# shg8/3DGS.cpp

Measured on AMD Instinct MI355X. Metric: frames/sec at 1920×1080, 1M Gaussians, higher is better.
Workload: dtype f32

## Files before the change

3dgs.cpp_amd/binding.py:

```python
import ctypes as C
import os

import numpy as np

_HERE = os.path.dirname(os.path.abspath(__file__))
LIB_PATH = os.environ.get("GS3D_HIP_LIB", os.path.join(_HERE, "libgs3d_hip.so"))

UNIFORMS_DT = np.dtype([("camera_position", "<f4", 4), ("proj_mat", "<f4", 16), ("view_mat", "<f4", 16),
                        ("width", "<u4"), ("height", "<u4"), ("tan_fovx", "<f4"), ("tan_fovy", "<f4")])
CAMERA_DT = np.dtype([("position", "<f4", 3), ("rotation", "<f4", 4), ("fov", "<f4"),
                      ("near_plane", "<f4"), ("far_plane", "<f4")])
VERTEX_FLOATS = 60
RECORD_FLOATS = 62
BLOB_PLANES = 59


KERNEL_SOURCES = ("gs_device.h", "gs_bin.h", "gs_scene.hip", "gs_preprocess.hip", "gs_radix.hip", "gs_bin_l1.hip", "gs_bin_l2.hip",
                  "gs_blend.hip", "gs_contrib.hip", "gs_features.hip", "gs_lift.hip", "gs_kernels.h")


def library_source_hash():
    import hashlib
    import re
    h = hashlib.sha256()
    for name in KERNEL_SOURCES + ("Makefile",):
        with open(os.path.join(_HERE, "csrc", name), "r") as f:
            text = f.read()
        if name != "Makefile":
            text = re.sub(r"/\*.*?\*/", " ", text, flags=re.S)
            text = re.sub(r"//[^\n]*", " ", text)
        else:
            text = re.sub(r"#[^\n]*", " ", text)
        h.update(name.encode() + b"\0" + " ".join(text.split()).encode())
    return h.hexdigest()


STAGES = dict(tiles=(0, np.uint32), depth=(1, np.float32), radius=(2, np.float32), aabb=(3, np.uint16),
              conic_opacity=(4, np.float32), uv_rg=(5, np.float32), b=(6, np.float32),
              depth_order=(7, np.uint32), alpha_cut=(8, np.float32), sorted_tile=(11, np.uint32), sorted_gid=(12, np.uint32),
              ranges=(13, np.uint32), lists_raw=(14, np.uint32), ranges_raw=(15, np.uint32))

SYMBOLS = ["gs_last_error", "gs_device_count", "gs_read_ply", "gs_activate_records", "gs_scene_load_ply", "gs_scene_from_records",
           "gs_scene_from_vertices", "gs_scene_from_device_blob", "gs_scene_blob_floats", "gs_scene_blob",
           "gs_scene_from_device_arrays", "gs_scene_update_from_device_arrays", "gs_debug_activation_expf_scan",
           "gs_scene_transform", "gs_transform_sh_matrices", "gs_transform_camera",
           "gs_scene_num_vertices", "gs_scene_quantize_sh", "gs_scene_sh_bits", "gs_scene_download_vertex_range",
           "gs_scene_download_vertices", "gs_scene_download_cov3d",
           "gs_deactivate_vertices", "gs_write_ply", "gs_scene_to_device_arrays", "gs_scene_download_records", "gs_scene_save_ply",
           "gs_scene_destroy", "gs_renderer_create", "gs_renderer_destroy", "gs_camera_uniforms",
           "gs_render", "gs_render_host", "gs_synchronize", "gs_set_timing", "gs_set_frames_in_flight", "gs_set_sort_path", "gs_set_exp_mode", "gs_set_graph_mode", "gs_set_blend_lockstep", "gs_get_blend_lockstep", "gs_set_level1_fused", "gs_get_level1_fused", "gs_set_blend_contraction", "gs_set_antialiased", "gs_get_antialiased", "gs_get_timing_totals",
           "gs_get_frame_intervals", "gs_get_stats", "gs_poll_stats", "gs_debug_download", "gs_accumulate_contributions", "gs_blend_features", "gs_lift_pixels", "gs_debug_expf_scan", "gs_debug_alpha_cut_scan", "gs_renderer_stream",
           "gs_dist_unique_id", "gs_dist_create", "gs_dist_rank", "gs_dist_world", "gs_dist_pose_count",
           "gs_dist_broadcast_scene", "gs_dist_broadcast_scene_ex", "gs_dist_verify", "gs_dist_destroy"]


class FrameStats(C.Structure):
    _fields_ = [("num_gaussians", C.c_uint64), ("num_visible", C.c_uint64), ("num_instances", C.c_uint64),
                ("instance_capacity", C.c_uint64), ("ms_preprocess", C.c_float), ("ms_prefix_sum", C.c_float),
                ("ms_preprocess_sort", C.c_float), ("ms_sort", C.c_float), ("ms_tile_boundary", C.c_float),
                ("ms_render", C.c_float), ("ms_total", C.c_float), ("retries", C.c_uint32),
                ("num_bin_entries", C.c_uint32), ("max_bin_entries", C.c_uint32), ("sort_path", C.c_uint32),
                ("bin_tiles", C.c_uint32), ("sort_level", C.c_uint32), ("blend_redo", C.c_uint32), ("blend_resolved", C.c_uint32), ("pad_", C.c_uint32)]

    def as_dict(self):
        return {k: getattr(self, k) for k, _ in self._fields_}


def debug_alpha_cut_scan(first_bits, count, device=0):
    bad, first = C.c_uint64(0), C.c_uint32(0)
    _check(lib().gs_debug_alpha_cut_scan(C.c_int(device), C.c_uint32(first_bits), C.c_uint64(count), C.byref(bad), C.byref(first)))
    return int(bad.value), (None if bad.value == 0 else int(first.value))


def debug_expf_scan(first_bits, count, device=0):
    blocks = (count + (1 << 20) - 1) >> 20
    sums = np.zeros(blocks, np.uint64)
    guard = np.zeros(4, np.float64)
    _check(lib().gs_debug_expf_scan(C.c_int(device), C.c_uint32(first_bits), C.c_uint64(count), _p(sums), C.c_uint64(blocks), _p(guard)))
    return sums, guard


def debug_activation_expf_scan(first_bits, count, device=0):
    blocks = (count + (1 << 20) - 1) >> 20
    sums = np.zeros(blocks, np.uint64)
    _check(lib().gs_debug_activation_expf_scan(C.c_int(device), C.c_uint32(first_bits), C.c_uint64(count), _p(sums), C.c_uint64(blocks)))
    return sums


class DeviceArrays(C.Structure):
    _fields_ = [("means", C.c_void_p), ("log_scales", C.c_void_p), ("quats", C.c_void_p), ("opacity_logits", C.c_void_p),
                ("sh_dc", C.c_void_p), ("sh_rest", C.c_void_p), ("sh_rest_coeffs", C.c_uint32)]


class Transform(C.Structure):
    _fields_ = [("rotation", C.c_float * 4), ("translation", C.c_float * 3), ("scale", C.c_float)]


def _transform(rotation, translation, scale):
    t = Transform()
    t.rotation[:] = [float(v) for v in rotation]
    t.translation[:] = [float(v) for v in translation]
    t.scale = float(scale)
    return t


def _tensor_rows(name, t, trailing, device):
    if not all(hasattr(t, a) for a in ("data_ptr", "shape", "dtype", "is_contiguous", "device")):
        raise TypeError(f"{name}: a device tensor is needed (data_ptr, shape, dtype, is_contiguous, device), got {type(t).__name__}")
    if str(t.dtype).rsplit(".", 1)[-1] != "float32":
        raise TypeError(f"{name}: dtype must be float32, not {t.dtype}")
    shape = tuple(int(d) for d in t.shape)
    if len(shape) < 1:
        raise ValueError(f"{name}: shape {shape} has no row axis")
    if not t.is_contiguous():
        raise ValueError(f"{name}: the tensor must be contiguous (dense rows); call .contiguous()")
    rows, rest = shape[0], tuple(d for d in shape[1:] if d != 1) if trailing is not None else shape[1:]
    if trailing is None:
        if len(rest) != 2 or rest[1] != 3 or rest[0] not in (0, 3, 8, 15):
            raise ValueError(f"{name}: shape {shape} is not (rows, k, 3) with k in 0, 3, 8, 15")
        rows = (rows, rest[0])
    elif rest != tuple(d for d in trailing if d != 1):
        raise ValueError(f"{name}: shape {shape} is not (rows, {', '.join(map(str, trailing))})")
    dev = t.device
    kind, index = getattr(dev, "type", str(dev).split(":")[0]), getattr(dev, "index", None)
    if kind == "cpu":
        raise ValueError(f"{name}: the tensor is on the CPU; Scene.from_records takes host data")
    if (0 if index is None else int(index)) != int(device):
        raise ValueError(f"{name}: the tensor is on device {index}, the scene on device {device}")
    return rows


def _device_arrays(tensors, device, require):
    trailing = dict(means=(3,), log_scales=(3,), quats=(4,), opacity_logits=(1,), sh_dc=(3,), sh_rest=None)
# ... 417 lines not shown
        elif out is not None:
            raise ValueError("out: an output for lifted values needs values")
        l.channels = channels
        if mask is not None:
            l.mask = _tensor_exact("mask", mask, ("uint8", "bool"), (h, w), dev, owner)
        shapes = dict(out=(n, channels), weight=(n,))
        members = dict(out="out", weight="out_weight")
        result = {}
        for name, t in asked.items():
            if t is None:
                continue
            if t is True:
                import torch
                t = torch.zeros(shapes[name], dtype=torch.float64, device=f"cuda:{int(dev)}")
            setattr(l, members[name], _tensor_exact(name, t, ("float64",), shapes[name], dev, owner))
            result[name] = t
        _complete_callers_work(values, mask, *result.values())
        _check(lib().gs_lift_pixels(self._h, C.byref(l)))
        return result

    def differentiable_feature_maps(self, features):
        return _feature_maps_function().apply(self, features)

    def render_host(self, uniforms, want_rgba=True, want_bgra=False):
        h, w = int(uniforms["height"][0]), int(uniforms["width"][0])
        rgba = np.zeros((h, w, 4), np.float32) if want_rgba else None
        bgra = np.zeros((h, w, 4), np.uint8) if want_bgra else None
        _check(lib().gs_render_host(self._h, _p(uniforms), _p(rgba) if want_rgba else None,
                                    _p(bgra) if want_bgra else None))
        self._frame_hw = (h, w)
        self._frames += 1
        return rgba, bgra

    def synchronize(self):
        _check(lib().gs_synchronize(self._h))

    def set_timing(self, enabled):
        _check(lib().gs_set_timing(self._h, C.c_int(int(enabled))))

    def set_frames_in_flight(self, frames):
        _check(lib().gs_set_frames_in_flight(self._h, C.c_int(int(frames))))

    def set_exp_mode(self, mode):
        _check(lib().gs_set_exp_mode(self._h, C.c_int(int(mode))))

    def set_blend_contraction(self, enabled):
        _check(lib().gs_set_blend_contraction(self._h, C.c_int(int(bool(enabled)))))

    def set_antialiased(self, enabled):
        _check(lib().gs_set_antialiased(self._h, C.c_int(int(bool(enabled)))))

    @property
    def antialiased(self):
        rc = lib().gs_get_antialiased(self._h)
        _check(min(rc, 0))
        return bool(rc)

    def set_fast_blend(self, fast):
        self.set_exp_mode(0 if fast else 2)
        self.set_blend_contraction(bool(fast))

    def set_graph_mode(self, enabled):
        _check(lib().gs_set_graph_mode(self._h, C.c_int(int(bool(enabled)))))

    def set_blend_lockstep(self, mode):
        _check(lib().gs_set_blend_lockstep(self._h, C.c_int(int(mode))))

    def blend_lockstep(self):
        settled = C.c_int(0)
        now = lib().gs_get_blend_lockstep(self._h, C.byref(settled))
        if now < 0:
            _check(now)
        return bool(now), bool(settled.value)

    def set_level1_fused(self, mode):
        _check(lib().gs_set_level1_fused(self._h, C.c_int(int(mode))))

    def level1_fused(self):
        now = lib().gs_get_level1_fused(self._h)
        if now < 0:
            _check(now)
        return bool(now)

    def set_sort_path(self, mode):
        _check(lib().gs_set_sort_path(self._h, C.c_int(int(mode))))

    def timing_totals(self, reset=True):
        st = FrameStats()
        n = C.c_uint64()
        _check(lib().gs_get_timing_totals(self._h, C.byref(st), C.byref(n), C.c_int(int(reset))))
        return st, n.value

    def frame_intervals(self, reset=True, capacity=8192):
        out = np.zeros(capacity, np.float32)
        n = C.c_uint64()
        _check(lib().gs_get_frame_intervals(self._h, _p(out), C.c_uint64(capacity), C.byref(n), C.c_int(int(reset))))
        return out[:min(capacity, n.value)].copy()

    def stats(self):
        st = FrameStats()
        _check(lib().gs_get_stats(self._h, C.byref(st)))
        return st

    def poll_stats(self):
        st = FrameStats()
        n = C.c_uint64()
        _check(lib().gs_poll_stats(self._h, C.byref(st), C.byref(n)))
        return st, n.value

    def stage(self, name, uniforms=None):
        code, dt = STAGES[name]
        st = self.stats()
        n, v, d = st.num_gaussians, st.num_visible, min(st.num_instances, st.instance_capacity)
        count = {"tiles": n, "depth": n, "radius": n, "aabb": 4 * n, "conic_opacity": 4 * n, "uv_rg": 4 * n,
                 "b": n, "alpha_cut": n, "depth_order": v, "sorted_tile": d, "sorted_gid": d, "lists_raw": d}.get(name)
        if name in ("ranges", "ranges_raw"):
            w, h = int(uniforms["width"][0]), int(uniforms["height"][0])
            count = 2 * ((w + 15) // 16) * ((h + 15) // 16)
        out = np.zeros(max(int(count), 1), dt)
        _check(lib().gs_debug_download(self._h, C.c_int(code), _p(out), C.c_uint64(int(count) * out.itemsize)))
        return out[:int(count)]

    @property
    def stream(self):
        return lib().gs_renderer_stream(self._h)

    def close(self):
        if self._h:
            lib().gs_renderer_destroy(self._h)
            self._h = None

    def __del__(self):
        try:
            self.close()
        except Exception:
            pass


class Dist:

    ID_BYTES = 128

    @staticmethod
    def unique_id():
        buf = (C.c_uint8 * Dist.ID_BYTES)()
        _check(lib().gs_dist_unique_id(buf))
        return bytes(buf)

    def __init__(self, unique_id, rank, world, device=0):
        h = C.c_void_p()
        buf = (C.c_uint8 * Dist.ID_BYTES).from_buffer_copy(unique_id)
        _check(lib().gs_dist_create(buf, C.c_int(rank), C.c_int(world), C.c_int(device), C.byref(h)))
        self._h = h
        lib().gs_dist_pose_count.restype = C.c_uint64

    @property
    def rank(self):
        return lib().gs_dist_rank(self._h)

    @property
    def world(self):
        return lib().gs_dist_world(self._h)

    def pose_count(self, poses):
        return int(lib().gs_dist_pose_count(self._h, C.c_uint64(poses)))

    def broadcast_scene(self, scene=None, root=0, copy_on_root=False):
        out = C.c_void_p()
        _check(lib().gs_dist_broadcast_scene_ex(self._h, scene._h if scene is not None else None, C.c_int(root),
                                                C.c_uint(1 if copy_on_root else 0), C.byref(out)))
        if scene is not None and out.value == scene._h.value:
            return scene
        return Scene(out)

    def close(self):
        if self._h:
            lib().gs_dist_destroy(self._h)
            self._h = None

    def __del__(self):
        try:
            self.close()
        except Exception:
            pass
```

3dgs.cpp_amd/csrc/gs_bin.h:

```cpp
#pragma once
#include "gs_device.h"

namespace gs {


template <int R>
__device__ __forceinline__ void cover_masks(int shift, int x0, int y0, int x1, int y1, uint64_t (&m)[R]) {
    const int W = 1 << shift;
    const int rows_per_word = 64 >> shift;
    const uint64_t rowbits = x1 > x0 ? ((x1 - x0 >= 64 ? ~0ull : ((1ull << (x1 - x0)) - 1ull)) << x0) : 0ull;
#pragma unroll
    for (int r = 0; r < R; ++r) {
        uint64_t w = 0;
        for (int yy = 0; yy < rows_per_word; ++yy) {
            const int y = r * rows_per_word + yy;
            if (y >= y0 && y < y1) w |= rowbits << (yy * W);
        }
        m[r] = w;
    }
}

template <int J>
__device__ __forceinline__ uint32_t lane_xor(uint32_t x) {
    if (J == 1) return (uint32_t)__builtin_amdgcn_mov_dpp((int)x, 0xB1, 0xF, 0xF, true);
// ... 74 lines not shown
    BinGrid g;
    const uint32_t* order;
    const uint32_t* n_items;
    uint32_t n_bound;
    const uint32_t* tiles;
    const ushort4* aabb;
    const float* depth;
    const uint4* vis;
    const uint32_t* vis_count;
    uint32_t vis_region_slots;
    uint32_t* hist;
    uint32_t* bin_count;
    uint32_t* cand;
    Counters* counters;
    uint32_t capacity;
    uint32_t nblk;
    uint64_t* stamps;
};

__device__ __forceinline__ bool bin_on_screen(const BinGrid& g, uint32_t bin) {
    return (bin & ((1u << g.grid_shift) - 1u)) < g.bins_x && (bin >> g.grid_shift) < g.bins_y;
}

__device__ __forceinline__ uint32_t l1_item(const L1Args& a, uint32_t p, uint32_t n, uint32_t& box_out) {
    uint32_t gid = 0;
    box_out = 0;
    if (p < n) {
        gid = a.order ? a.order[p] : p;
        if (a.tiles[gid] != 0) {
            const ushort4 box = a.aabb[gid];
            const uint32_t x0 = box.x >> a.g.bin_shift, y0 = box.y >> a.g.bin_shift;
            const uint32_t x1 = ((box.z - 1u) >> a.g.bin_shift) + 1u, y1 = ((box.w - 1u) >> a.g.bin_shift) + 1u;
            box_out = x0 | (y0 << 8) | (x1 << 16) | (y1 << 24);
        }
    }
    return gid;
}
__device__ __forceinline__ uint32_t l1_vis_block(const L1Args& a, uint32_t blk, uint32_t& first) {
    const uint32_t per = a.vis_region_slots / kL1Items, region = blk / per, at = (blk % per) * kL1Items;
    uint32_t cnt = (uint32_t)__builtin_amdgcn_readfirstlane((int)a.vis_count[region * kVisCounterStride]);
    if (cnt > a.vis_region_slots) cnt = a.vis_region_slots;
    first = region * a.vis_region_slots + at;
    return cnt > at ? (cnt - at < (uint32_t)kL1Items ? cnt - at : (uint32_t)kL1Items) : 0u;
}
__device__ __forceinline__ uint32_t l1_bin_box(const L1Args& a, uint4 r) {
    const uint32_t x0 = (r.z & 0xFFFFu) >> a.g.bin_shift, y0 = (r.z >> 16) >> a.g.bin_shift;
    const uint32_t x1 = (((r.w & 0xFFFFu) - 1u) >> a.g.bin_shift) + 1u, y1 = (((r.w >> 16) - 1u) >> a.g.bin_shift) + 1u;
    return x0 | (y0 << 8) | (x1 << 16) | (y1 << 24);
}
template <int R>
__device__ __forceinline__ void packed_cover_masks(int shift, uint32_t box, uint64_t (&m)[R]) {
    cover_masks<R>(shift, (int)(box & 255u), (int)((box >> 8) & 255u), (int)((box >> 16) & 255u), (int)(box >> 24), m);
}

__device__ __forceinline__ uint64_t cover_word(int shift, uint32_t box, int r) {
    const int x0 = (int)(box & 255u), y0 = (int)((box >> 8) & 255u), x1 = (int)((box >> 16) & 255u), y1 = (int)(box >> 24);
    const int W = 1 << shift, rows_per_word = 64 >> shift;
    const uint64_t rowbits = x1 > x0 ? (((1ull << (x1 - x0)) - 1ull) << x0) : 0ull;
    uint64_t w = 0;
    for (int yy = 0; yy < rows_per_word; ++yy) {
        const int y = r * rows_per_word + yy;
        if (y >= y0 && y < y1) w |= rowbits << (yy * W);
    }
    return w;
}

constexpr uint32_t kL1XcdRun = 32;
__host__ __device__ constexpr uint32_t l1_grid(uint32_t nblk) {
    return (nblk + 8u * kL1XcdRun - 1u) / (8u * kL1XcdRun) * (8u * kL1XcdRun);
}
__device__ __forceinline__ uint32_t l1_block() {
    const uint32_t xcd = blockIdx.x & 7u, j = blockIdx.x >> 3;
    return ((j / kL1XcdRun) * 8u + xcd) * kL1XcdRun + j % kL1XcdRun;
}

constexpr int kCandWords = 3;
__device__ __forceinline__ uint32_t bin_local_box16(const BinGrid& g, uint32_t bin, ushort4 box) {
    const int S = 1 << g.bin_shift;
    const int ox = (int)(bin & ((1u << g.grid_shift) - 1u)) << g.bin_shift, oy = (int)(bin >> g.grid_shift) << g.bin_shift;
    const int lx0 = max((int)box.x, ox) - ox, ly0 = max((int)box.y, oy) - oy;
    const int lx1 = min((int)box.z, ox + S) - ox - 1, ly1 = min((int)box.w, oy + S) - oy - 1;
    return (uint32_t)lx0 | ((uint32_t)ly0 << 4) | ((uint32_t)lx1 << 8) | ((uint32_t)ly1 << 12);
}

}
```

3dgs.cpp_amd/csrc/gs_bin_l1.hip:

```cpp
#include "gs_bin.h"

namespace gs {

template <int R1>
__global__ __launch_bounds__(BLOCK) void k_l1_hist(L1Args a) {
    constexpr int NB = 64 * R1;
    __shared__ uint32_t s_hist[NB];
    __shared__ uint32_t s_vis;
    const int tid = threadIdx.x, lane = tid & (WAVE - 1), w = tid / WAVE;
    frame_stamp(a.stamps, ST_L1_COUNT);
    const uint32_t blk = l1_block();
    if (blk >= a.nblk) return;
    uint32_t n = a.n_items ? *a.n_items : a.n_bound;
    if (n > a.n_bound) n = a.n_bound;
    uint32_t vis_first = 0;
    const uint32_t vis_here = a.vis ? l1_vis_block(a, blk, vis_first) : 0u;
    if (a.vis && vis_here == 0) return;
    for (int b = tid; b < NB; b += BLOCK) s_hist[b] = 0;
    if (tid == 0) s_vis = 0;
    __syncthreads();
    __shared__ uint32_t s_box[kL1Chunks][WAVE];
    {
        uint32_t box[kL1PerWave];
        if (a.vis) {
// ... 183 lines not shown
            if (__builtin_amdgcn_ballot_w64(mr != 0) == 0) continue;
            walk_column(wave_transpose64(mr, lane), s_start[r * 64 + lane] + s_cnt[ch][r * 64 + lane], out, s_ids[ch]);
        }
    }
}

template <int R1>
__global__ __launch_bounds__(BLOCK) void k_l1_scatter_any_order(L1Args a) {
    constexpr int NB = 64 * R1;
    __shared__ uint32_t s_cur[NB];
    __shared__ uint32_t scratch[8];
    const int tid = threadIdx.x, lane = tid & (WAVE - 1), w = tid / WAVE;
    frame_stamp(a.stamps, ST_L1_SCATTER);
    const uint32_t blk = l1_block();
    if (blk >= a.nblk) return;
    uint32_t vis_first = 0;
    const uint32_t vis_here = a.vis ? l1_vis_block(a, blk, vis_first) : 0u;
    if (a.vis && blk != 0 && vis_here == 0) return;
    {
        uint32_t c[NB / BLOCK], sum = 0;
#pragma unroll
        for (int k = 0; k < NB / BLOCK; ++k) {
            c[k] = a.bin_count[tid * (NB / BLOCK) + k];
            sum += c[k];
        }
        uint32_t total;
        uint32_t off = block_excl_scan<BLOCK>(sum, scratch, &total);
#pragma unroll
        for (int k = 0; k < NB / BLOCK; ++k) {
            const uint32_t b = tid * (NB / BLOCK) + k;
            s_cur[b] = off + (bin_on_screen(a.g, b) ? a.hist[(size_t)b * a.nblk + blk] : 0u);
            if (blk == 0) a.bin_count[kBinOffsets + b] = off;
            off += c[k];
            if (blk == 0 && c[k]) atomicMax(&a.counters->max_bin, c[k]);
        }
        if (blk == 0 && tid == 0) {
            a.counters->bin_entries = total;
            if (total > a.capacity) atomicOr(&a.counters->overflow, 1u);
        }
    }
    uint32_t nt[kL1PerWave], key[kL1PerWave], ids[kL1PerWave];
    ushort4 tb[kL1PerWave];
    if (a.vis) {
        uint4 r[kL1PerWave];
#pragma unroll
        for (int j = 0; j < kL1PerWave; ++j) {
            const uint32_t q = (w * kL1PerWave + j) * WAVE + lane;
            r[j] = q < vis_here ? a.vis[vis_first + q] : make_uint4(0, 0, 0, 0);
        }
#pragma unroll
        for (int j = 0; j < kL1PerWave; ++j) {
            const uint32_t q = (w * kL1PerWave + j) * WAVE + lane;
            nt[j] = q < vis_here ? 1u : 0u;
            ids[j] = r[j].x;
            key[j] = r[j].y;
            tb[j] = make_ushort4((unsigned short)(r[j].z & 0xFFFFu), (unsigned short)(r[j].z >> 16), (unsigned short)(r[j].w & 0xFFFFu),
                                 (unsigned short)(r[j].w >> 16));
        }
    } else {
#pragma unroll
        for (int j = 0; j < kL1PerWave; ++j) {
            const uint32_t p = blk * kL1Items + (w * kL1PerWave + j) * WAVE + lane;
            nt[j] = p < a.n_bound ? a.tiles[p] : 0u;
            ids[j] = p;
        }
#pragma unroll
        for (int j = 0; j < kL1PerWave; ++j) {
            const uint32_t p = blk * kL1Items + (w * kL1PerWave + j) * WAVE + lane;
            tb[j] = make_ushort4(0, 0, 0, 0);
            key[j] = 0;
            if (nt[j] != 0) {
                tb[j] = a.aabb[p];
                key[j] = __float_as_uint(a.depth[p]);
            }
        }
    }
    __syncthreads();
    auto emit = [&](uint32_t bin, uint32_t k, uint32_t gid, ushort4 box) {
        const uint32_t pos = atomicAdd(&s_cur[bin], 1u);
        if (pos < a.capacity) {
            uint32_t* const rec = a.cand + (size_t)kCandWords * pos;
            rec[0] = k;
            rec[1] = gid;
            rec[2] = bin_local_box16(a.g, bin, box);
        }
    };
#pragma unroll
    for (int j = 0; j < kL1PerWave; ++j) {
        const uint32_t gid = ids[j];
        uint32_t x0 = 0, y0 = 0, x1 = 0, y1 = 0;
        if (nt[j] != 0) {
            x0 = tb[j].x >> a.g.bin_shift, y0 = tb[j].y >> a.g.bin_shift;
            x1 = ((tb[j].z - 1u) >> a.g.bin_shift) + 1u, y1 = ((tb[j].w - 1u) >> a.g.bin_shift) + 1u;
        }
        const bool big = (x1 - x0) * (y1 - y0) > kL1BigBox;
        if (!big)
            for (uint32_t y = y0; y < y1; ++y)
                for (uint32_t x = x0; x < x1; ++x) emit((y << a.g.grid_shift) | x, key[j], gid, tb[j]);
        for (uint64_t bm = __ballot(big); bm != 0; bm &= bm - 1) {
            const int src = __ffsll((unsigned long long)bm) - 1;
            const uint32_t bx0 = (uint32_t)__builtin_amdgcn_readlane((int)x0, src), by0 = (uint32_t)__builtin_amdgcn_readlane((int)y0, src);
            const uint32_t bw = (uint32_t)__builtin_amdgcn_readlane((int)x1, src) - bx0;
            const uint32_t cells = bw * ((uint32_t)__builtin_amdgcn_readlane((int)y1, src) - by0);
            const uint32_t bkey = (uint32_t)__builtin_amdgcn_readlane((int)key[j], src);
            const uint32_t bgid = (uint32_t)__builtin_amdgcn_readlane((int)gid, src);
            const uint32_t blo = (uint32_t)__builtin_amdgcn_readlane((int)((uint32_t)tb[j].x | ((uint32_t)tb[j].y << 16)), src);
            const uint32_t bhi = (uint32_t)__builtin_amdgcn_readlane((int)((uint32_t)tb[j].z | ((uint32_t)tb[j].w << 16)), src);
            const ushort4 bbox = make_ushort4((unsigned short)(blo & 0xFFFFu), (unsigned short)(blo >> 16), (unsigned short)(bhi & 0xFFFFu),
                                              (unsigned short)(bhi >> 16));
            for (uint32_t c = lane; c < cells; c += WAVE) emit(((by0 + c / bw) << a.g.grid_shift) | (bx0 + c % bw), bkey, bgid, bbox);
        }
    }
}

__global__ __launch_bounds__(BLOCK) void k_vis_to_planes(const uint4* __restrict__ vis, const uint32_t* __restrict__ vis_count,
                                                         uint32_t region_slots, uint32_t* __restrict__ tiles, float* __restrict__ depth,
                                                         ushort4* __restrict__ aabb) {
    const uint32_t region = blockIdx.y, slot = blockIdx.x * BLOCK + threadIdx.x;
    const uint32_t count = min(vis_count[region * kVisCounterStride + 1], region_slots);
    if (slot >= count) return;
    const uint4 e = vis[(size_t)region * region_slots + slot];
    const uint32_t x0 = e.z & 0xFFFFu, y0 = e.z >> 16, x1 = e.w & 0xFFFFu, y1 = e.w >> 16;
    tiles[e.x] = (x1 - x0) * (y1 - y0);
    depth[e.x] = __uint_as_float(e.y);
    aabb[e.x] = make_ushort4((unsigned short)x0, (unsigned short)y0, (unsigned short)x1, (unsigned short)y1);
}
void launch_vis_to_planes(const AttrView& av, uint32_t n, hipStream_t s) {
    if (!av.vis || n == 0) return;
    (void)hipMemsetAsync(av.tiles, 0, (size_t)n * sizeof(uint32_t), s);
    hipLaunchKernelGGL(k_vis_to_planes, dim3((av.vis_region_slots + BLOCK - 1) / BLOCK, kVisRegions), dim3(BLOCK), 0, s, av.vis, av.vis_count,
                       av.vis_region_slots, av.tiles, av.depth, av.aabb);
}

static L1Args l1_args(const BinLaunch& b) {
    L1Args a;
    a.g = BinGrid{b.tiles_x, b.tiles_y, b.bins_x, b.bins_y, b.bin_shift, b.grid_shift};
    a.order = b.order;
    a.n_items = b.n_items;
    a.n_bound = b.n_bound;
    a.tiles = b.tiles;
    a.aabb = b.aabb;
    a.depth = b.depth;
    a.vis = b.vis;
    a.vis_count = b.vis_count;
    a.vis_region_slots = b.vis_region_slots;
    a.hist = b.hist;
    a.bin_count = b.bin_count;
    a.cand = b.cand;
    a.counters = b.counters;
    a.capacity = b.cand_capacity;
    a.nblk = b.vis ? kVisRegions * (b.vis_region_slots / kL1Items) : bin_level1_blocks(b.n_bound);
    a.stamps = b.stamps;
    return a;
}

uint32_t bin_level1_blocks(uint32_t n_items) { return (n_items + kL1Items - 1) / kL1Items; }
uint32_t vis_region_slots(uint32_t n) {
    const uint32_t groups = (n + BLOCK - 1) / BLOCK, per_region = (groups + kVisRegions - 1) / kVisRegions;
    const uint32_t slots = per_region * BLOCK;
    return slots == 0 ? kL1Items : (slots + kL1Items - 1) / kL1Items * kL1Items;
}
uint32_t bin_level1_columns(uint32_t n_items) {
    const uint32_t dense = kVisRegions * (vis_region_slots(n_items) / kL1Items), planes = bin_level1_blocks(n_items);
    return dense > planes ? dense : planes;
}
static_assert(BLOCK >= (int)kVisRegions, "k_blend's first workgroup zeroes the list counters, k_l1_scan's sums them: a thread each");

// ... 22 lines not shown
```

3dgs.cpp_amd/csrc/gs_bin_l2.hip:

```cpp
#include "gs_bin.h"

namespace gs {

struct SlabDesc {
    uint32_t off, c_total;
    uint32_t kmin;
    int32_t sh;
    uint32_t b_lo, b_hi;
    uint32_t ready;
    uint32_t pad;
    uint32_t cur[64];
};
static_assert(sizeof(SlabDesc) == 288, "descriptor layout");

struct BuildArgs {
    BinGrid g;
    uint32_t* cand;
    const uint32_t* bin_count;
    const float* depth;
    const ushort4* aabb;
    uint32_t* ranges;
    uint32_t* sorted_gid;
    Counters* counters;
    uint32_t capacity;
    uint32_t cand_capacity;
    SlabDesc* slabs;
    uint32_t slab_capacity;
    uint32_t epoch;
    uint64_t* stamps;
    const uint32_t* l1_words;
    uint32_t l1_cap;
};

__device__ __forceinline__ uint32_t bin_candidates(const BuildArgs& a, uint32_t bin) {
    return a.l1_words ? a.l1_words[(size_t)(kL1FusedCursor0 + bin) * kL1FusedStride] : a.bin_count[bin];
}
__device__ __forceinline__ uint32_t bin_offset(const BuildArgs& a, uint32_t bin) {
    return a.l1_words ? ((bin >> a.g.grid_shift) * a.g.bins_x + (bin & ((1u << a.g.grid_shift) - 1u))) * a.l1_cap : a.bin_count[kBinOffsets + bin];
}
__device__ __forceinline__ void bin_close_one_pass(const BuildArgs& a, uint32_t& c, int tid) {
    if (!a.l1_words) return;
    if (tid == 0 && c != 0) {
        atomicAdd(&a.counters->bin_entries, c);
        atomicMax(&a.counters->max_bin, c);
    }
    if (c > a.l1_cap) {
        if (tid == 0) atomicOr(&a.counters->overflow, 1u);
        c = 0;
    }
}
__device__ __forceinline__ void one_pass_visible(const BuildArgs& a) {
    if (!a.l1_words || blockIdx.x != 0 || threadIdx.x >= kVisRegions) return;
    uint32_t v = a.l1_words[(size_t)threadIdx.x * kL1FusedStride];
    for (int o = WAVE / 2; o != 0; o >>= 1) v += (uint32_t)__shfl_xor((int)v, o);
    if ((threadIdx.x & (WAVE - 1)) == 0 && v != 0) atomicAdd(&a.counters->visible, v);
}

__device__ __forceinline__ uint32_t bin_local_box(const BinGrid& g, uint32_t bin, ushort4 box) {
    const int S = 1 << g.bin_shift;
    const int ox = (int)(bin & ((1u << g.grid_shift) - 1u)) << g.bin_shift, oy = (int)(bin >> g.grid_shift) << g.bin_shift;
    const int lx0 = max((int)box.x, ox) - ox, ly0 = max((int)box.y, oy) - oy;
    const int lx1 = min((int)box.z, ox + S) - ox, ly1 = min((int)box.w, oy + S) - oy;
    return (uint32_t)lx0 | ((uint32_t)ly0 << 8) | ((uint32_t)lx1 << 16) | ((uint32_t)ly1 << 24);
}

constexpr int kBuildSlots = 16;

#ifdef GS_BUILD_TIMING
__device__ unsigned long long g_build_t[1024][10];
#define BUILD_ROW(v) uint32_t build_row = (v)
#define BUILD_ROW_SET(v) build_row = (v)
#define BUILD_T(i) do { if (threadIdx.x == 0) g_build_t[build_row][i] = wall_clock64(); } while (0)
#else
#define BUILD_ROW(v) do { } while (0)
#define BUILD_ROW_SET(v) do { } while (0)
#define BUILD_T(i) do { } while (0)
#endif

template <int R2, int THREADS, bool SORT>
struct BuildLayout {
    static constexpr int NW = THREADS / WAVE;
    static constexpr int MAXC = SORT ? THREADS * 16 : 0;
    static constexpr int SS = 64 * R2;
    static constexpr bool CACHE_BOX = SORT && R2 <= 4;
    static constexpr int TABLES = 3 * SS + kBuildSlots * SS / 2 + (SORT ? 0 : kBuildSlots * WAVE);
    static constexpr int WCNT = SORT ? NW * 256 : 0;
    static constexpr int T_OFF = (SORT && (CACHE_BOX || TABLES > MAXC)) ? 2 * MAXC : 0;
    static constexpr int WORDS = (T_OFF + TABLES > 2 * MAXC + WCNT) ? T_OFF + TABLES : 2 * MAXC + WCNT;
};

template <int R2, int THREADS, bool SORT>
__global__ __launch_bounds__(THREADS) void k_bin_build(BuildArgs a) {
    frame_stamp(a.stamps, ST_L2);
    one_pass_visible(a);
    BUILD_ROW(blockIdx.x);
    using L = BuildLayout<R2, THREADS, SORT>;
    constexpr int NW = L::NW, MAXC = L::MAXC, SS = L::SS, PER = kBuildSlots / NW;
    extern __shared__ uint32_t smem[];
    uint32_t* const s_key = smem;
    uint32_t* const s_id = smem + MAXC;
    uint32_t (*const s_wcnt)[256] = reinterpret_cast<uint32_t(*)[256]>(smem + 2 * MAXC);
    uint32_t* const t_cnt = smem + L::T_OFF;
    uint32_t* const t_cur = t_cnt + SS;
    uint16_t (*const r_cnt)[SS] = reinterpret_cast<uint16_t(*)[SS]>(t_cnt + 3 * SS);
    uint32_t* const w_ids = t_cnt + 3 * SS + kBuildSlots * SS / 2;
    __shared__ uint32_t scratch[NW];
    __shared__ uint32_t s_seg;

    const int tid = threadIdx.x, lane = tid & (WAVE - 1), w = tid / WAVE;
    const uint32_t bin = ((blockIdx.x / a.g.bins_x) << a.g.grid_shift) | (blockIdx.x % a.g.bins_x);
    BUILD_T(0);
    uint32_t c, off;
    c = bin_candidates(a, bin);
    off = bin_offset(a, bin);
// ... 198 lines not shown
    for (uint32_t rb = 0; rb < nch; rb += kBuildSlots, par ^= 1) {
        uint64_t col[PER][R2];
#pragma unroll
        for (int j = 0; j < PER; ++j) {
            const int slot = w * PER + j;
            uint32_t gid;
            chunk_columns(rb + slot, col[j], gid);
#pragma unroll
            for (int r = 0; r < R2; ++r) r_cnt[slot][r * 64 + lane] = (uint16_t)__popcll(col[j][r]);
            if (!SORT) w_ids[slot * WAVE + lane] = gid;
        }
        __syncthreads();
        for (int t = tid; t < SS; t += THREADS) {
            uint32_t run = 0;
#pragma unroll
            for (int k = 0; k < kBuildSlots; ++k) {
                const uint32_t v = r_cnt[k][t];
                r_cnt[k][t] = (uint16_t)run;
                run += v;
            }
            t_cur[(par ^ 1) * SS + t] = t_cur[par * SS + t] + run;
        }
        __syncthreads();
#pragma unroll
        for (int j = 0; j < PER; ++j) {
            const int slot = w * PER + j;
            const uint32_t ch = rb + slot;
            const uint32_t* ids = SORT ? s_id + (ch < nch ? ch : 0u) * WAVE : w_ids + slot * WAVE;
#pragma unroll
            for (int r = 0; r < R2; ++r) {
                if (__builtin_amdgcn_ballot_w64(col[j][r] != 0) == 0) continue;
                walk_column(col[j][r], t_cur[par * SS + r * 64 + lane] + r_cnt[slot][r * 64 + lane], out, ids);
            }
        }
    }
    BUILD_T(7);
}

#ifdef GS_BUILD_TIMING
extern "C" int gs_debug_build_timing(unsigned long long* out ) {
    return hipMemcpyFromSymbol(out, HIP_SYMBOL(g_build_t), sizeof(unsigned long long) * 1024 * 10) == hipSuccess ? 0 : -1;
}
#endif

__device__ __forceinline__ __amdgpu_buffer_rsrc_t uniform_rsrc(const void* p, uint32_t bytes) {
    const uint64_t addr = reinterpret_cast<uint64_t>(p);
    const uint32_t lo = (uint32_t)__builtin_amdgcn_readfirstlane((int)(uint32_t)addr);
    const uint32_t hi = (uint32_t)__builtin_amdgcn_readfirstlane((int)(uint32_t)(addr >> 32));
    return __builtin_amdgcn_make_buffer_rsrc(reinterpret_cast<void*>(((uint64_t)hi << 32) | lo), 0,
                                             __builtin_amdgcn_readfirstlane((int)bytes), 0x27000);
}

__device__ __forceinline__ uint32_t cover16(uint32_t pb) {
    const uint32_t lx0 = pb & 15u, ly0 = (pb >> 4) & 15u, lx1 = (pb >> 8) & 15u, ly1 = (pb >> 12) & 15u;
    const uint32_t xm = ((2u << lx1) - (1u << lx0)) & 15u;
    const uint32_t rows = (16u << (4u * ly1)) - (1u << (4u * ly0));
    return (xm * 0x1111u) & rows;
}

template <int ROUNDS>
struct FastLayout {
    static constexpr int THREADS = 1024, NW = THREADS / WAVE, MAXC = THREADS * ROUNDS;
    static constexpr int WCNT_WORDS = NW * 512 / 2;
    static constexpr int MISC_WORDS = 64 + 64 + NW * 64;
    static constexpr int TAIL = WCNT_WORDS > MISC_WORDS ? WCNT_WORDS : MISC_WORDS;
    static constexpr int WORDS = 2 * MAXC + TAIL;
};

template <int ROUNDS, int MODE = 0>
__device__ __forceinline__ void bin_fast_body(const BuildArgs& a) {
    constexpr bool SLABS = MODE != 0;
    using L = FastLayout<ROUNDS>;
    constexpr int THREADS = L::THREADS, NW = L::NW, MAXC = L::MAXC;
    extern __shared__ uint32_t smem[];
    uint32_t* const s_pay = smem;
    uint32_t* const s_key = smem + MAXC;
    uint16_t (*const s_wcnt)[512] = reinterpret_cast<uint16_t(*)[512]>(smem + 2 * MAXC);
    uint32_t* const s_id = smem + MAXC;
    uint16_t* const s_box = reinterpret_cast<uint16_t*>(smem);
    uint16_t (*const s_tbl)[64] = reinterpret_cast<uint16_t(*)[64]>(smem + MAXC / 2);
    uint32_t* const t_cnt = smem + 2 * MAXC;
    uint32_t* const t_cur = t_cnt + 64;
    uint32_t (*const s_seg)[64] = reinterpret_cast<uint32_t(*)[64]>(t_cnt + 128);
    __shared__ uint32_t scratch[NW], scratch_hi[NW];
    __shared__ uint32_t s_seg0, s_flag;
    constexpr int kSlotBits = SLABS ? 16 : 14;
    constexpr uint32_t kSlotMask = (1u << kSlotBits) - 1u;
    constexpr uint32_t kMaxInBin = SLABS ? 65535u : (uint32_t)MAXC;
    constexpr int kMaxSlabs = 16;
    __shared__ uint32_t g_cur[SLABS ? 64 : 1], t_tot[SLABS ? 64 : 1];
    __shared__ uint32_t slab_first[SLABS ? kMaxSlabs + 1 : 1];
    __shared__ uint32_t cnt2[(MODE == 1 || MODE == 3) ? kMaxSlabs : 1][64];
    __shared__ uint32_t s_fill;
    __shared__ uint16_t q_order[MODE == 3 ? 1024 : 1];
    __shared__ uint32_t q_item, q_planned;

    BUILD_ROW(MODE == 2 ? 1023u : blockIdx.x);
    if constexpr (MODE != 2) frame_stamp(a.stamps, ST_L2);
    if constexpr (MODE != 2) one_pass_visible(a);
    int tid = threadIdx.x, lane = tid & (WAVE - 1), w = tid / WAVE;
    auto screen_bin = [&](uint32_t i) { return ((i / a.g.bins_x) << a.g.grid_shift) | (i % a.g.bins_x); };
    uint32_t bin = screen_bin(MODE == 3 ? 0u : blockIdx.x);
    bool slab_item = MODE == 2;
    BUILD_T(0);
    uint32_t c_total = 0, off = 0;
    auto bin_extent = [&]() {
        c_total = (uint32_t)__builtin_amdgcn_readfirstlane((int)bin_candidates(a, bin));
        off = (uint32_t)__builtin_amdgcn_readfirstlane((int)bin_offset(a, bin));
        bin_close_one_pass(a, c_total, tid);
        if ((uint64_t)off + c_total > a.cand_capacity) c_total = 0;
        if (c_total > kMaxInBin) {
            if (tid == 0) atomicOr(&a.counters->overflow, 2u);
            c_total = 0;
        }
    };
    if constexpr (MODE == 0 || MODE == 1) bin_extent();
    if (tid == 0) s_flag = 0;
    BUILD_T(1);
#define multi (MODE == 2 ? true : (MODE == 1 ? c_total > (uint32_t)MAXC : (MODE == 3 ? (slab_item || c_total > (uint32_t)MAXC) : false)))
    uint32_t c = multi ? 0u : c_total;
    int rounds = (int)((c + THREADS - 1) / THREADS);
    typedef uint32_t u32x3 __attribute__((ext_vector_type(3)));
#define recs uniform_rsrc(a.cand + (size_t)kCandWords * off, c_total * 12u)
    uint64_t lt_mask = (1ull << lane) - 1ull;
    uint32_t wbase = (uint32_t)w * (uint32_t)rounds * WAVE;
    auto refresh = [&]() {
        int t = threadIdx.x;
        asm volatile("" : "+v"(t));
        tid = t;
        lane = t & (WAVE - 1);
        w = t / WAVE;
        lt_mask = (1ull << lane) - 1ull;
        wbase = (uint32_t)w * (uint32_t)rounds * WAVE;
    };
    auto radix_pass = [&](int shift, int db, uint32_t sub) {
        const uint32_t dmask = (1u << db) - 1u;
        for (int k = tid; k < NW * 512 / 2; k += THREADS) reinterpret_cast<uint32_t*>(&s_wcnt[0][0])[k] = 0;
        __syncthreads();
        uint32_t key[ROUNDS], pay[ROUNDS], rank[ROUNDS];
#pragma unroll
        for (int r = 0; r < ROUNDS; ++r) {
            key[r] = 0;
            pay[r] = 0;
            rank[r] = 0;
            if (r < rounds) {
                const uint32_t e = wbase + r * WAVE + lane;
                const bool ok = e < c;
                if (ok) {
                    key[r] = s_key[e] - sub;
                    pay[r] = s_pay[e];
                }
                const uint32_t d = (key[r] >> shift) & dmask;
                const uint64_t okm = __ballot(ok);
                uint32_t mlo = (uint32_t)okm, mhi = (uint32_t)(okm >> 32);
#pragma unroll
                for (int bit = 0; bit < 9; ++bit) {
                    if (bit < db) {
                        const uint32_t mine = (d >> bit) & 1u;
                        const uint64_t b = __builtin_amdgcn_ballot_w64(mine != 0);
                        const uint32_t splat = 0u - mine;
                        mlo &= ~((uint32_t)b ^ splat);
                        mhi &= ~((uint32_t)(b >> 32) ^ splat);
                    }
                }
                const uint64_t m = ((uint64_t)mhi << 32) | mlo;
                uint32_t old = 0;
                const int leader = m ? (__ffsll((unsigned long long)m) - 1) : 0;
                if (ok && lane == leader) {
                    old = s_wcnt[w][d];
                    s_wcnt[w][d] = (uint16_t)(old + (uint32_t)__popcll(m));
                }
                old = __shfl(old, leader, WAVE);
                rank[r] = old + (uint32_t)__popcll(m & lt_mask);
            }
        }
        __syncthreads();
        {
            uint32_t cw[NW], cnt = 0;
            if (tid < 512) {
#pragma unroll
                for (int k = 0; k < NW; ++k) {
                    cw[k] = s_wcnt[k][tid];
                    cnt += cw[k];
                }
            }
            uint32_t all;
            uint32_t excl = block_excl_scan<THREADS>(cnt, scratch, &all);
            if (tid < 512) {
#pragma unroll
                for (int k = 0; k < NW; ++k) {
                    s_wcnt[k][tid] = (uint16_t)excl;
                    excl += cw[k];
                }
            }
        }
        __syncthreads();
#pragma unroll
        for (int r = 0; r < ROUNDS; ++r) {
            if (r < rounds) {
                const uint32_t e = wbase + r * WAVE + lane;
                if (e < c) {
                    const uint32_t d = (key[r] >> shift) & dmask;
                    const uint32_t pos = (uint32_t)s_wcnt[w][d] + rank[r];
                    s_key[pos] = key[r];
                    s_pay[pos] = pay[r];
                }
            }
        }
        __syncthreads();
    };
    auto block_minmax = [&](uint32_t lo, uint32_t hi, uint32_t& kmin, uint32_t& span) {
#pragma unroll
        for (int d = 1; d < WAVE; d <<= 1) {
            lo = min(lo, (uint32_t)__shfl_xor((int)lo, d, WAVE));
            hi = max(hi, (uint32_t)__shfl_xor((int)hi, d, WAVE));
        }
        __syncthreads();
        if (lane == 0) {
            scratch[w] = lo;
            scratch_hi[w] = hi;
        }
        __syncthreads();
#pragma unroll
        for (int k = 0; k < NW; ++k) {
            lo = min(lo, scratch[k]);
            hi = max(hi, scratch_hi[k]);
        }
        kmin = (uint32_t)__builtin_amdgcn_readfirstlane((int)lo);
        span = (uint32_t)__builtin_amdgcn_readfirstlane((int)hi) - kmin;
    };
    auto key_range = [&](uint32_t& kmin, uint32_t& span) {
        uint32_t lo = 0xFFFFFFFFu, hi = 0u;
#pragma unroll
        for (int r = 0; r < ROUNDS; ++r) {
            const uint32_t e = r * THREADS + tid;
            if (r < rounds && e < c) {
                const uint32_t k = s_key[e];
                lo = min(lo, k);
                hi = max(hi, k);
            }
        }
        block_minmax(lo, hi, kmin, span);
    };
    auto sort_by_key_lsd = [&](uint32_t kmin, uint32_t span) {
        const int bits = span ? 32 - __builtin_clz(span) : 0;
        const int npass = (bits + 8) / 9;
        const int db = npass ? (bits + npass - 1) / npass : 0;
#pragma unroll 1
        for (int pass = 0; pass < npass; ++pass) radix_pass(pass * db, db, pass == 0 ? kmin : 0u);
        return npass ? kmin : 0u;
    };
    constexpr uint32_t kMsdBuckets = 4096, kMsdBucketMax = 64;
    uint32_t* const m_cnt = smem + 2 * MAXC;
    uint16_t* const m_start = reinterpret_cast<uint16_t*>(smem + 2 * MAXC + kMsdBuckets / 2);
    static_assert(kMsdBuckets * 4 <= L::TAIL * 4, "the bucket tables live in the counters' area");
    auto sort_by_key_msd = [&](uint32_t kmin, uint32_t span) -> bool {
        const int bits = 32 - __builtin_clz(span);
        const int sh = bits > 12 ? bits - 12 : 0;
        for (uint32_t k = tid; k < kMsdBuckets / 2; k += THREADS) m_cnt[k] = 0;
        __syncthreads();
        uint32_t key[ROUNDS], pay[ROUNDS];
#pragma unroll
        for (int r = 0; r < ROUNDS; ++r) {
            const uint32_t e = r * THREADS + tid;
            key[r] = 0;
            pay[r] = 0;
            if (r < rounds && e < c) {
                key[r] = s_key[e];
                pay[r] = s_pay[e];
                const uint32_t b = (key[r] - kmin) >> sh;
                atomicAdd(&m_cnt[b >> 1], 1u << (16u * (b & 1u)));
            }
        }
        __syncthreads();
        {
            const uint2 w2 = reinterpret_cast<const uint2*>(m_cnt)[tid];
            const uint32_t v0 = w2.x & 0xFFFFu, v1 = w2.x >> 16, v2 = w2.y & 0xFFFFu, v3 = w2.y >> 16;
            uint32_t all;
            uint32_t excl = block_excl_scan<THREADS>(v0 + v1 + v2 + v3, scratch, &all);
            if (max(max(v0, v1), max(v2, v3)) > kMsdBucketMax) s_flag = 2;
            reinterpret_cast<uint2*>(m_cnt)[tid] = make_uint2(0u, 0u);
            ushort4 st;
            st.x = (unsigned short)excl;
            st.y = (unsigned short)(excl + v0);
            st.z = (unsigned short)(excl + v0 + v1);
            st.w = (unsigned short)(excl + v0 + v1 + v2);
            reinterpret_cast<ushort4*>(m_start)[tid] = st;
        }
        __syncthreads();
        if (__builtin_amdgcn_readfirstlane((int)s_flag) == 2) {
            __syncthreads();
            if (tid == 0) s_flag = 0;
            return false;
        }
#pragma unroll
        for (int r = 0; r < ROUNDS; ++r) {
            const uint32_t e = r * THREADS + tid;
            if (r < rounds && e < c) {
                const uint32_t b = (key[r] - kmin) >> sh;
                const uint32_t old = atomicAdd(&m_cnt[b >> 1], 1u << (16u * (b & 1u)));
                const uint32_t pos = (uint32_t)m_start[b] + ((old >> (16u * (b & 1u))) & 0xFFFFu);
                s_key[pos] = key[r];
                s_pay[pos] = pay[r];
            }
        }
        __syncthreads();
        uint32_t dst[ROUNDS];
#pragma unroll
        for (int r = 0; r < ROUNDS; ++r) {
            const uint32_t e = r * THREADS + tid;
            dst[r] = 0xFFFFFFFFu;
            if (r < rounds && e < c) {
                const uint32_t k = s_key[e];
                pay[r] = s_pay[e];
                key[r] = k;
                const uint32_t b = (k - kmin) >> sh;
                const uint32_t j0 = m_start[b], j1 = b + 1 < kMsdBuckets ? (uint32_t)m_start[b + 1] : c;
                uint32_t before = 0;
                for (uint32_t j = j0; j < j1; ++j) {
                    const uint32_t kj = s_key[j];
                    before += (kj < k || (kj == k && j < e)) ? 1u : 0u;
                }
                dst[r] = j0 + before;
            }
        }
        __syncthreads();
#pragma unroll
        for (int r = 0; r < ROUNDS; ++r)
            if (dst[r] != 0xFFFFFFFFu) {
                s_key[dst[r]] = key[r];
                s_pay[dst[r]] = pay[r];
            }
        __syncthreads();
        return true;
    };
    auto sort_by_key = [&](bool try_msd) -> uint32_t {
        uint32_t kmin, span;
        key_range(kmin, span);
        if (span == 0) return 0u;
        if constexpr (ROUNDS <= 12) {
            if (try_msd && sort_by_key_msd(kmin, span)) return 0u;
        }
        return sort_by_key_lsd(kmin, span);
    };
    const int S = 1 << a.g.bin_shift;
    auto place_lists = [&](uint32_t v, uint32_t* cursors) {
        uint32_t d_bin;
        const uint32_t excl = block_excl_scan<THREADS>(v, scratch, &d_bin);
        if (tid == 0) {
            const uint32_t seg = d_bin ? atomicAdd(&a.counters->instances, d_bin) : 0u;
            s_seg0 = seg;
            if ((uint64_t)seg + d_bin > a.capacity) atomicOr(&a.counters->overflow, 1u);
        }
        __syncthreads();
        if (tid < 64) {
            const uint32_t ox = (bin & ((1u << a.g.grid_shift) - 1u)) << a.g.bin_shift, oy = (bin >> a.g.grid_shift) << a.g.bin_shift;
            const uint32_t lx = (uint32_t)tid & (uint32_t)(S - 1), ly = (uint32_t)tid >> a.g.bin_shift;
            const uint32_t x = ox + lx, y = oy + ly;
            const uint64_t start64 = (uint64_t)s_seg0 + excl;
            const uint32_t start = start64 > a.capacity ? a.capacity : (uint32_t)start64;
            const uint32_t end = start64 + v > a.capacity ? a.capacity : (uint32_t)(start64 + v);
            if (ly < (uint32_t)S && x < a.g.tiles_x && y < a.g.tiles_y) {
                a.ranges[2 * (y * a.g.tiles_x + x)] = v ? start : 0u;
                a.ranges[2 * (y * a.g.tiles_x + x) + 1] = v ? end : 0u;
            }
            cursors[tid] = start;
        }
    };
    uint32_t n_slabs = 1, g_kmin = 0;
    int g_sh = 0;
    auto plan_bin = [&]() {
    if constexpr (MODE == 1 || MODE == 3) if (!slab_item && multi) {
        uint32_t lo = 0xFFFFFFFFu, hi = 0u;
        for (uint32_t base = 0; base < c_total; base += 8 * THREADS) {
            uint32_t k[8];
#pragma unroll
            for (int r = 0; r < 8; ++r) k[r] = __builtin_amdgcn_raw_buffer_load_b32(recs, (base + r * THREADS + tid) * 12u, 0, 0);
#pragma unroll
            for (int r = 0; r < 8; ++r)
                if (base + r * THREADS + tid < c_total) {
                    lo = min(lo, k[r]);
                    hi = max(hi, k[r]);
                }
        }
        uint32_t span;
        block_minmax(lo, hi, g_kmin, span);
        const int bits = span ? 32 - __builtin_clz(span) : 0;
        g_sh = bits > 12 ? bits - 12 : 0;
        for (uint32_t k = tid; k < kMsdBuckets / 2; k += THREADS) m_cnt[k] = 0;
        for (uint32_t k = tid; k < (uint32_t)kMaxSlabs * 64u; k += THREADS) cnt2[k >> 6][k & 63u] = 0;
        __syncthreads();
        for (uint32_t base = 0; base < c_total; base += 8 * THREADS) {
            uint32_t k[8];
#pragma unroll
            for (int r = 0; r < 8; ++r) k[r] = __builtin_amdgcn_raw_buffer_load_b32(recs, (base + r * THREADS + tid) * 12u, 0, 0);
#pragma unroll
            for (int r = 0; r < 8; ++r)
                if (base + r * THREADS + tid < c_total) {
                    const uint32_t bk = (k[r] - g_kmin) >> g_sh;
                    atomicAdd(&m_cnt[bk >> 1], 1u << (16u * (bk & 1u)));
                }
        }
        __syncthreads();
        {
            const uint2 w2 = reinterpret_cast<const uint2*>(m_cnt)[tid];
            const uint32_t v0 = w2.x & 0xFFFFu, v1 = w2.x >> 16, v2 = w2.y & 0xFFFFu, v3 = w2.y >> 16;
            uint32_t all;
            const uint32_t excl = block_excl_scan<THREADS>(v0 + v1 + v2 + v3, scratch, &all);
            if (max(max(v0, v1), max(v2, v3)) > (uint32_t)MAXC) s_flag = 3;
            ushort4 st;
            st.x = (unsigned short)excl;
            st.y = (unsigned short)(excl + v0);
            st.z = (unsigned short)(excl + v0 + v1);
            st.w = (unsigned short)(excl + v0 + v1 + v2);
            reinterpret_cast<ushort4*>(m_start)[tid] = st;
            if (tid == 0) {
                slab_first[0] = 0;
                s_fill = 1;
            }
        }
        __syncthreads();
        for (int k = 0; k < kMaxSlabs; ++k) {
            const uint32_t base = m_start[slab_first[k]];
            if (c_total - base <= (uint32_t)MAXC) break;
#pragma unroll
            for (int j = 0; j < 4; ++j) {
                const uint32_t bk = 4u * tid + j;
                const uint32_t p0 = m_start[bk], p1 = bk + 1 < kMsdBuckets ? (uint32_t)m_start[bk + 1] : c_total;
                if (p0 - base <= (uint32_t)MAXC && p1 - base > (uint32_t)MAXC && bk > slab_first[k]) {
                    slab_first[k + 1] = bk;
                    s_fill = k + 2;
                }
            }
            __syncthreads();
            if (s_fill != (uint32_t)k + 2) {
// ... 59 lines not shown
        }
        __syncthreads();
        place_lists(tid < 64 ? t_tot[tid] : 0u, g_cur);
        __syncthreads();
        if (tid == 0) {
            const uint32_t base = n_slabs ? atomicAdd(&a.counters->slabs, n_slabs) : 0u;
            s_seg0 = base;
            if (base + n_slabs > a.slab_capacity) atomicOr(&a.counters->overflow, 2u);
        }
        __syncthreads();
        const uint32_t dbase = (uint32_t)__builtin_amdgcn_readfirstlane((int)s_seg0);
        if (dbase + n_slabs <= a.slab_capacity) {
            auto put = [&](uint32_t* p, uint32_t v) {
                if constexpr (MODE == 3) __hip_atomic_store(p, v, __ATOMIC_RELAXED, __HIP_MEMORY_SCOPE_AGENT);
                else *p = v;
            };
            for (uint32_t k = 0; k < n_slabs; ++k) {
                SlabDesc* d = a.slabs + dbase + k;
                if (tid < 64) put(&d->cur[tid], g_cur[tid] + cnt2[k][tid]);
                if (tid == 64) {
                    put(&d->off, off);
                    put(&d->c_total, c_total);
                    put(&d->kmin, g_kmin);
                    put(reinterpret_cast<uint32_t*>(&d->sh), (uint32_t)g_sh);
                    put(&d->b_lo, slab_first[k]);
                    put(&d->b_hi, slab_first[k + 1]);
                }
            }
            if constexpr (MODE == 3) {
                asm volatile("s_waitcnt vmcnt(0)" ::: "memory");
                __syncthreads();
                if (tid == 0) {
                    for (uint32_t k = 0; k < n_slabs; ++k)
                        __hip_atomic_store(&a.slabs[dbase + k].ready, a.epoch, __ATOMIC_RELAXED, __HIP_MEMORY_SCOPE_AGENT);
                    asm volatile("s_waitcnt vmcnt(0)" ::: "memory");
                }
            }
        }
        n_slabs = 0;
    }
    };
    if constexpr (MODE == 1) plan_bin();
    auto slab_body = [&](const uint32_t slab) {
    if constexpr (SLABS) if (multi) {
        const uint32_t b_lo = slab_first[slab], b_hi = slab_first[slab + 1];
        __syncthreads();
        if (tid == 0) s_fill = 0;
        __syncthreads();
        for (uint32_t base = 0; base < c_total; base += 8 * THREADS) {
            uint32_t k[8], bx[8];
#pragma unroll
            for (int r = 0; r < 8; ++r) {
                const u32x3 rec = __builtin_amdgcn_raw_buffer_load_b96(recs, (base + r * THREADS + tid) * 12u, 0, 0);
                k[r] = rec.x;
                bx[r] = rec.z;
            }
#pragma unroll
            for (int r = 0; r < 8; ++r) {
                const uint32_t e = base + r * THREADS + tid;
                const uint32_t bk = (k[r] - g_kmin) >> g_sh;
                const bool mine = e < c_total && bk >= b_lo && bk < b_hi;
                const uint64_t mm = __builtin_amdgcn_ballot_w64(mine);
                if (mm != 0) {
                    uint32_t at = 0;
                    if (lane == __ffsll((unsigned long long)mm) - 1) at = atomicAdd(&s_fill, (uint32_t)__popcll(mm));
                    at = (uint32_t)__builtin_amdgcn_readlane((int)at, __ffsll((unsigned long long)mm) - 1) + (uint32_t)__popcll(mm & lt_mask);
                    if (mine && at < (uint32_t)MAXC) {
                        s_key[at] = k[r];
                        s_pay[at] = e | (bx[r] << kSlotBits);
                    }
                }
            }
        }
        __syncthreads();
        c = min((uint32_t)__builtin_amdgcn_readfirstlane((int)s_fill), (uint32_t)MAXC);
        rounds = (int)((c + THREADS - 1) / THREADS);
        wbase = (uint32_t)w * (uint32_t)rounds * WAVE;
    }
    for (int attempt = 0; c != 0 && attempt < 2; ++attempt) {
        uint32_t tid12 = (uint32_t)tid * 12u;
        asm volatile("" : "+v"(tid12));
        constexpr int HR = ROUNDS <= 8 ? ROUNDS : ROUNDS / 2;
        const int h_end = multi ? 0 : ROUNDS;
#pragma unroll
        for (int h = 0; h < h_end; h += HR) {
            uint32_t k[HR], b[HR];
#pragma unroll
            for (int r = 0; r < HR; ++r) {
                k[r] = 0;
                b[r] = 0;
                if (h + r < rounds) {
                    const u32x3 rec = __builtin_amdgcn_raw_buffer_load_b96(recs, tid12 + (uint32_t)(h + r) * (THREADS * 12u), 0, 0);
                    k[r] = rec.x;
                    b[r] = rec.z;
                }
            }
#pragma unroll
            for (int r = 0; r < HR; ++r) {
                const uint32_t e = (h + r) * THREADS + tid;
                if (h + r < rounds && e < c) {
                    s_key[e] = k[r];
                    s_pay[e] = e | (b[r] << kSlotBits);
                }
            }
        }
        if (attempt == 0) BUILD_T(2);
        sort_by_key(attempt == 0);
        if (attempt == 0) BUILD_T(8);
        refresh();
        uint32_t my_id[ROUNDS], run_len[(ROUNDS + 3) / 4];
        bool too_long = false;
#pragma unroll
        for (int q = 0; q < (ROUNDS + 3) / 4; ++q) run_len[q] = 0;
#pragma unroll
        for (int r = 0; r < ROUNDS; ++r) {
            const uint32_t e = r * THREADS + tid;
            my_id[r] = 0;
            if (r < rounds && e < c) {
                my_id[r] = __builtin_amdgcn_raw_buffer_load_b32(recs, (s_pay[e] & kSlotMask) * 12u + 4u, 0, 0);
                const uint32_t k = s_key[e];
                if (attempt == 0 && (e == 0 || s_key[e - 1] != k) && e + 1 < c && s_key[e + 1] == k) {
                    uint32_t more = 1;
                    while (e + more + 1 < c && more < 64 && s_key[e + more + 1] == k) ++more;
                    if (e + more + 1 < c && s_key[e + more + 1] == k) too_long = true;
                    run_len[r / 4] |= more << (8 * (r % 4));
                }
            }
        }
        if (too_long) s_flag = 1;
        __syncthreads();
        const bool redo = __builtin_amdgcn_readfirstlane((int)s_flag) != 0;
#pragma unroll
        for (int r = 0; r < ROUNDS; ++r) {
            const uint32_t e = r * THREADS + tid;
            if (r < rounds && e < c) s_id[e] = my_id[r];
        }
        __syncthreads();
        if (attempt == 0) BUILD_T(9);
        if (multi && redo) {
            if (tid == 0) atomicOr(&a.counters->overflow, 2u);
            __syncthreads();
            if (tid == 0) s_flag = 0;
            break;
        }
        if (!redo) {
#pragma unroll
            for (int r = 0; r < ROUNDS; ++r) {
                const uint32_t more = (run_len[r / 4] >> (8 * (r % 4))) & 255u;
                if (more != 0) {
                    const uint32_t e = r * THREADS + tid;
                    for (uint32_t i = e + 1; i <= e + more; ++i) {
                        const uint32_t vi = s_id[i], vp = s_pay[i];
                        uint32_t j = i;
                        while (j > e && s_id[j - 1] > vi) {
                            s_id[j] = s_id[j - 1];
                            s_pay[j] = s_pay[j - 1];
                            --j;
                        }
                        s_id[j] = vi;
                        s_pay[j] = vp;
                    }
                }
            }
            __syncthreads();
            break;
        }
        const uint32_t id_base = sort_by_key(false);
        uint32_t nk[ROUNDS], ni[ROUNDS], nb[ROUNDS];
#pragma unroll
        for (int r = 0; r < ROUNDS; ++r) {
            const uint32_t e = r * THREADS + tid;
            nk[r] = ni[r] = nb[r] = 0;
            if (r < rounds && e < c) {
                const uint32_t pw = s_pay[e];
                nk[r] = __builtin_amdgcn_raw_buffer_load_b32(recs, (pw & kSlotMask) * 12u, 0, 0);
                ni[r] = s_id[e] + id_base;
                nb[r] = pw >> kSlotBits;
            }
        }
        __syncthreads();
#pragma unroll
        for (int r = 0; r < ROUNDS; ++r) {
            const uint32_t e = r * THREADS + tid;
            if (r < rounds && e < c) {
                u32x3 rec = {nk[r], ni[r], nb[r]};
                __builtin_amdgcn_raw_buffer_store_b96(rec, recs, e * 12u, 0, 0);
            }
        }
        __threadfence_block();
        if (tid == 0) s_flag = 0;
        __syncthreads();
    }
#undef recs
    BUILD_T(3);
    refresh();
    const uint32_t nch = (c + WAVE - 1) / WAVE;
    {
        uint32_t pb16[ROUNDS];
#pragma unroll
        for (int r = 0; r < ROUNDS; ++r) {
            const uint32_t e = r * THREADS + tid;
            pb16[r] = e < c ? s_pay[e] >> kSlotBits : 0u;
        }
        __syncthreads();
        for (uint32_t k = tid; k < (uint32_t)MAXC / 2; k += THREADS) smem[MAXC / 2 + k] = 0;
        if (tid < 64) t_cnt[tid] = 0;
        __syncthreads();
#pragma unroll
        for (int r = 0; r < ROUNDS; ++r) {
            const uint32_t e = r * THREADS + tid;
            const uint32_t pb = pb16[r];
            if (e < c) s_box[e] = (uint16_t)pb;
            if (S == 4) {
                const uint32_t ch = (uint32_t)r * NW + (uint32_t)__builtin_amdgcn_readfirstlane(w);
                if (ch < nch) {
                    const uint32_t cm = e < c ? cover16(pb) : 0u;
                    uint32_t mine = 0;
#pragma unroll
                    for (int t = 0; t < 16; ++t) {
                        const uint64_t bal = __builtin_amdgcn_ballot_w64(((cm >> t) & 1u) != 0);
                        mine = lane == t ? (uint32_t)__popcll(bal) : mine;
                    }
                    s_tbl[ch][lane] = (uint16_t)mine;
                }
            }
        }
        if (S != 4) {
            __syncthreads();
            for (uint32_t ch = w; ch < nch; ch += NW) {
                const uint32_t e = ch * WAVE + lane;
                const uint32_t pb = e < c ? (uint32_t)s_box[e] : 0xFFFFu;
                uint64_t m[1];
                cover_masks<1>(3, (int)(pb & 15u), (int)((pb >> 4) & 15u), (int)((pb >> 8) & 15u) + 1, (int)(pb >> 12) + 1, m);
                if (e >= c) m[0] = 0;
                s_tbl[ch][lane] = (uint16_t)__popcll(wave_transpose64(m[0], lane));
            }
        }
    }
    __syncthreads();
    BUILD_T(4);
    {
        const int t = tid & 63, g = tid >> 6;
        const uint32_t per = (nch + NW - 1) / NW;
        const uint32_t q0 = min(nch, (uint32_t)g * per), q1 = min(nch, q0 + per);
        uint32_t sum = 0;
        for (uint32_t q = q0; q < q1; ++q) sum += s_tbl[q][t];
        s_seg[g][t] = sum;
        __syncthreads();
        if (tid < 64) {
            uint32_t run = 0;
#pragma unroll
            for (int k = 0; k < NW; ++k) {
                const uint32_t v = s_seg[k][tid];
                s_seg[k][tid] = run;
                run += v;
            }
            t_cnt[tid] = run;
        }
        __syncthreads();
        uint32_t run = s_seg[g][t];
// ... 163 lines not shown
    BUILD_T(7);
}
#undef multi
template <int ROUNDS> __global__ void k_bin_fast(BuildArgs a);
template <> __global__ __launch_bounds__(1024, 4) void k_bin_fast<4>(BuildArgs a) { bin_fast_body<4>(a); }
template <> __global__ __launch_bounds__(1024, 4) void k_bin_fast<8>(BuildArgs a) { bin_fast_body<8>(a); }
template <> __global__ __launch_bounds__(1024, 4) void k_bin_fast<12>(BuildArgs a) { bin_fast_body<12>(a); }
template <> __global__ __launch_bounds__(1024, 4) void k_bin_fast<16>(BuildArgs a) { bin_fast_body<16>(a); }
constexpr int kSlabRounds = 12;
__global__ __launch_bounds__(1024, 4) void k_bin_slabs(BuildArgs a) { bin_fast_body<kSlabRounds, 1>(a); }
__global__ __launch_bounds__(1024, 4) void k_slab_work(BuildArgs a) { bin_fast_body<kSlabRounds, 2>(a); }
__global__ __launch_bounds__(1024, 4) void k_bin_queue(BuildArgs a) { bin_fast_body<kSlabRounds, 3>(a); }

template <int R2, int THREADS, bool SORT>
static hipError_t build_prepare() {
    return hipFuncSetAttribute(reinterpret_cast<const void*>(&k_bin_build<R2, THREADS, SORT>),
                               hipFuncAttributeMaxDynamicSharedMemorySize,
                               (int)(BuildLayout<R2, THREADS, SORT>::WORDS * sizeof(uint32_t)));
}
template <int ROUNDS>
static hipError_t fast_prepare() {
    return hipFuncSetAttribute(reinterpret_cast<const void*>(&k_bin_fast<ROUNDS>), hipFuncAttributeMaxDynamicSharedMemorySize,
                               (int)(FastLayout<ROUNDS>::WORDS * sizeof(uint32_t)));
}
void bin_debug_occupancy() {
    int n4 = -1, n8 = -1, n16 = -1;
    (void)hipOccupancyMaxActiveBlocksPerMultiprocessor(&n4, reinterpret_cast<const void*>(&k_bin_fast<4>), 1024,
                                                       FastLayout<4>::WORDS * sizeof(uint32_t));
    (void)hipOccupancyMaxActiveBlocksPerMultiprocessor(&n8, reinterpret_cast<const void*>(&k_bin_fast<8>), 1024,
                                                       FastLayout<8>::WORDS * sizeof(uint32_t));
    (void)hipOccupancyMaxActiveBlocksPerMultiprocessor(&n16, reinterpret_cast<const void*>(&k_bin_fast<16>), 1024,
                                                       FastLayout<16>::WORDS * sizeof(uint32_t));
    hipFuncAttributes a4{}, a8{};
    (void)hipFuncGetAttributes(&a4, reinterpret_cast<const void*>(&k_bin_fast<4>));
    (void)hipFuncGetAttributes(&a8, reinterpret_cast<const void*>(&k_bin_fast<8>));
    std::fprintf(stderr, "[occupancy] k_bin_fast<4>: %d blocks/CU (regs %d, static lds %zu, dyn %zu); <8>: %d (regs %d); <16>: %d\n", n4,
                 a4.numRegs, a4.sharedSizeBytes, FastLayout<4>::WORDS * sizeof(uint32_t), n8, a8.numRegs, n16);
}

hipError_t bin_prepare_device() {
    hipError_t e = build_prepare<4, 1024, true>();
    if (e == hipSuccess) e = build_prepare<16, 1024, true>();
    if (e == hipSuccess) e = fast_prepare<8>();
    if (e == hipSuccess) e = fast_prepare<12>();
    if (e == hipSuccess) e = fast_prepare<16>();
    if (e == hipSuccess)
        e = hipFuncSetAttribute(reinterpret_cast<const void*>(&k_bin_slabs), hipFuncAttributeMaxDynamicSharedMemorySize,
                                (int)(FastLayout<kSlabRounds>::WORDS * sizeof(uint32_t)));
    if (e == hipSuccess)
        e = hipFuncSetAttribute(reinterpret_cast<const void*>(&k_slab_work), hipFuncAttributeMaxDynamicSharedMemorySize,
                                (int)(FastLayout<kSlabRounds>::WORDS * sizeof(uint32_t)));
    if (e == hipSuccess)
        e = hipFuncSetAttribute(reinterpret_cast<const void*>(&k_bin_queue), hipFuncAttributeMaxDynamicSharedMemorySize,
                                (int)(FastLayout<kSlabRounds>::WORDS * sizeof(uint32_t)));
    return e;
}

template <int R2>
static void launch_build(const BuildArgs& a, bool sort, uint32_t bins, hipStream_t s) {
    constexpr size_t lds1 = BuildLayout<R2, 1024, true>::WORDS * sizeof(uint32_t);
    constexpr size_t lds2 = BuildLayout<R2, 1024, false>::WORDS * sizeof(uint32_t);
    if (sort) hipLaunchKernelGGL((k_bin_build<R2, 1024, true>), dim3(bins), dim3(1024), lds1, s, a);
    else hipLaunchKernelGGL((k_bin_build<R2, 1024, false>), dim3(bins), dim3(1024), lds2, s, a);
}

void launch_bin_level2(const BinLaunch& b, int level, hipStream_t s) {
    BuildArgs a;
    a.g = BinGrid{b.tiles_x, b.tiles_y, b.bins_x, b.bins_y, b.bin_shift, b.grid_shift};
    a.cand = b.cand;
    a.bin_count = b.bin_count;
    a.depth = b.depth;
    a.aabb = b.aabb;
    a.ranges = b.ranges;
    a.sorted_gid = b.sorted_gid;
    a.counters = b.counters;
    a.capacity = b.capacity;
    a.cand_capacity = b.cand_capacity;
    a.slabs = reinterpret_cast<SlabDesc*>(b.slabs);
    a.slab_capacity = b.slab_capacity;
    a.epoch = b.slab_epoch;
    a.stamps = b.stamps;
    a.l1_words = b.l1_fused_words;
    a.l1_cap = b.l1_fused_cap;
    const uint32_t bins = b.bins_x * b.bins_y;
    const bool sort = level < kBinSortLevels;
    if (sort && b.bin_shift <= 3) {
        if (level == 0) hipLaunchKernelGGL(k_bin_fast<4>, dim3(bins), dim3(1024), FastLayout<4>::WORDS * sizeof(uint32_t), s, a);
        else if (level == 1) hipLaunchKernelGGL(k_bin_fast<8>, dim3(bins), dim3(1024), FastLayout<8>::WORDS * sizeof(uint32_t), s, a);
        else if (level == 2) hipLaunchKernelGGL(k_bin_fast<12>, dim3(bins), dim3(1024), FastLayout<12>::WORDS * sizeof(uint32_t), s, a);
        else if (level == 3) hipLaunchKernelGGL(k_bin_fast<16>, dim3(bins), dim3(1024), FastLayout<16>::WORDS * sizeof(uint32_t), s, a);
        else if (b.slab_epoch != 0) {
            hipLaunchKernelGGL(k_bin_queue, dim3(bins < kQueueWorkGroups ? bins : kQueueWorkGroups), dim3(1024), FastLayout<kSlabRounds>::WORDS * sizeof(uint32_t), s, a);
        } else {
            hipLaunchKernelGGL(k_bin_slabs, dim3(bins), dim3(1024), FastLayout<kSlabRounds>::WORDS * sizeof(uint32_t), s, a);
            hipLaunchKernelGGL(k_slab_work, dim3(kSlabWorkGroups), dim3(1024), FastLayout<kSlabRounds>::WORDS * sizeof(uint32_t), s, a);
        }
    } else if (b.bin_shift <= 3) {
        launch_build<1>(a, sort, bins, s);
    } else if (b.bin_shift == 4) {
        launch_build<4>(a, sort, bins, s);
    } else {
        launch_build<16>(a, sort, bins, s);
    }
}
}
```

3dgs.cpp_amd/csrc/gs_kernels.h:

```cpp
#pragma once
#include <hip/hip_runtime.h>
#include <stdint.h>

#include "../../include/gs3d_hip.h"
#include "gs_levels.h"

namespace gs {

constexpr int kSortTileKeys = 2048;
constexpr int kSortMaxBlocks = 1024;

enum ScenePlane { P_POS = 0, P_SCALE = 3, P_ROT = 6, P_OPACITY = 10, P_SH = 11, P_COUNT = 59 };
constexpr uint64_t blob_stride(uint64_t n) { return (n + 15) & ~uint64_t(15); }
constexpr uint64_t blob_floats(uint64_t n) { return P_SH * blob_stride(n) + 48 * n; }

struct SceneView {
    const float* blob;
    const float* cov3d;
    uint32_t n;
    uint32_t stride;
    const uint16_t* sh16;
    const float* acut;
    const uint32_t* perm;
};

struct AttrRecord {
    float4 conic_op;
    float4 uv_rg;
    float4 b_cut_r;
    float4 depth_radius;
};
static_assert(sizeof(AttrRecord) == 64, "one line per Gaussian");

struct AttrView {
    uint32_t* tiles;
    float* depth;
    ushort4* aabb;
    AttrRecord* rec;
    uint4* vis;
    uint32_t* vis_count;
    uint32_t vis_region_slots;
};
constexpr uint32_t kVisRegions = 256, kVisCounterStride = 32;
uint32_t vis_region_slots(uint32_t n);

constexpr uint32_t kL1FusedStride = 32, kL1FusedCursor0 = kVisRegions, kL1FusedWords = (kVisRegions + 1024) * kL1FusedStride;
struct L1Fused {
    uint32_t* words;
    uint32_t* cand;
    uint32_t cap;
    uint64_t* vis_mask;
    uint32_t tiles_x, tiles_y, bins_x, bins_y;
    int bin_shift, grid_shift;
};

struct Counters {
    uint32_t visible;
    uint32_t instances;
    uint32_t overflow;
    uint32_t bin_entries;
    uint32_t max_bin;
    uint32_t slabs;
    uint32_t blend_resolved;
    uint32_t blend_redo;
    uint32_t q_head, q_bins_done;
};
enum FrameStamp { ST_PREPROCESS = 0, ST_ORDER = 1, ST_L1_COUNT = 2, ST_L1_SCATTER = 3, ST_L2 = 4, ST_BLEND = 5, ST_END = 6, ST_COUNT = 8 };

struct FrameParams {
    gs_uniforms u;
    float* rgba;
    uint8_t* bgra;
    Counters* host_counters;
    uint64_t* host_stamps;
};

constexpr int kBinSortMax = 16384;
constexpr uint32_t kSlabDescBytes = 288, kSlabCapacity = 8192, kSlabWorkGroups = 512, kQueueWorkGroups = 256;

void launch_cov3d(const float* blob, float* cov3d, uint32_t n, uint32_t stride, uint32_t first, uint32_t count, hipStream_t s);
void launch_alpha_cut(const float* blob, float* cut, uint32_t n, uint32_t stride, uint32_t* beyond_unit, hipStream_t s);
void launch_permute_blob(const float* src, const uint32_t* perm, float* dst, uint32_t n, uint32_t stride, hipStream_t s);
void launch_blob_checksum(const float* blob, uint64_t floats, uint64_t* out, hipStream_t s);
void launch_sh_to_half(const float* blob, uint16_t* sh16, uint32_t stride, uint32_t first, uint32_t count, hipStream_t s);
void launch_ingest_arrays(const gs_device_arrays& a, float* blob, uint32_t stride, uint32_t first, uint32_t count, bool replace_rest,
                          hipStream_t s);
struct SceneTransform {
    float R[9];
    float t[3];
    float s;
    float q[4];
    float M[9 + 25 + 49];
};
void launch_scene_transform(const SceneTransform& x, float* blob, uint32_t stride, uint32_t first, uint32_t count, hipStream_t s);
void launch_scene_export(const gs_device_arrays_out& a, const float* blob, uint32_t stride, uint32_t first, uint32_t count, hipStream_t s);
void launch_scene_export_records(float* records, const float* blob, uint32_t stride, uint32_t first, uint32_t count, hipStream_t s);
void launch_preprocess(const SceneView& sv, const gs_uniforms& u, const AttrView& av, Counters* counters,
                       const FrameParams* fp, uint64_t* stamps, bool antialiased, const L1Fused& lf, hipStream_t s);
void launch_frame_end(uint64_t* stamps, uint64_t* host_stamps, const FrameParams* fp, uint32_t* l1_words, uint32_t l1_counters, hipStream_t s);

struct RadixPass {
    const uint32_t* keys_in;
    const uint32_t* vals_in;
    uint32_t* keys_out;
    uint32_t* vals_out;
    const uint32_t* n_in;
    uint32_t n_static;
    const uint32_t* tiles;
    uint32_t* n_out;
    uint32_t* block_hist;
    uint32_t* digit_total;
    int shift;
    int bits;
    int blocks;
    int first;
    uint64_t* stamps;
};
void launch_radix_pass(const RadixPass& p, hipStream_t s);

struct BinLaunch {
    const uint32_t* order;
    const uint32_t* n_items;
    uint32_t n_bound;
    const uint32_t* tiles;
    const ushort4* aabb;
    const float* depth;
    const uint4* vis;
    uint32_t* vis_count;
    uint32_t vis_region_slots;
    uint32_t* hist;
    uint32_t* bin_count;
    uint32_t* cand;
    uint32_t* ranges;
    uint32_t* sorted_gid;
    Counters* counters;
    uint32_t capacity;
    uint32_t cand_capacity;
    const uint32_t* l1_fused_words;
    uint32_t l1_fused_cap;
    void* slabs;
    uint32_t slab_capacity;
    uint32_t slab_epoch;
    uint32_t tiles_x, tiles_y, bins_x, bins_y;
    int bin_shift;
    int grid_shift;
    uint64_t* stamps;
};
void launch_vis_to_planes(const AttrView& av, uint32_t n, hipStream_t s);
void launch_records_to_planes(const uint64_t* vis_mask, const uint32_t* perm, const AttrView& av, uint32_t n, uint32_t width, uint32_t height,
                              hipStream_t s);
uint32_t bin_level1_blocks(uint32_t n_items);
uint32_t bin_level1_columns(uint32_t n_items);
void bin_debug_occupancy();
hipError_t bin_prepare_device();
void launch_bin_level1_count(const BinLaunch& b, hipStream_t s);
void launch_bin_level1_scatter(const BinLaunch& b, bool any_order, hipStream_t s);
void launch_bin_level2(const BinLaunch& b, int level, hipStream_t s);

void launch_blend(const uint32_t* ranges, const uint32_t* sorted_gid, const uint32_t* tile_order, const AttrView& av,
                  uint32_t width,
                  uint32_t height, float* rgba, uint8_t* bgra, Counters* counters,
                  Counters* host_counters ,
                  int exp_mode ,
                  bool contract ,
                  const FrameParams* fp,
                  bool lockstep ,
                  uint64_t* stamps ,
                  hipStream_t s);

void launch_contributions(const uint32_t* ranges, const uint32_t* sorted_gid, const uint32_t* tile_order, const AttrRecord* rec,
                          uint32_t width, uint32_t height, const uint8_t* mask, uint64_t* weight, uint32_t* pixels, uint32_t* top_id,
                          hipStream_t s);

constexpr int kFeatureGroup = 16;
void launch_features(const uint32_t* ranges, const uint32_t* sorted_gid, const uint32_t* tile_order, const AttrRecord* rec,
                     uint32_t width, uint32_t height, const float* features, uint32_t channels, float* out_features, float* out_alpha,
                     float* out_depth, float* out_median, hipStream_t s);

constexpr int kLiftGroup = 16, kLiftGroupSmall = 4;
void launch_lift(const uint32_t* ranges, const uint32_t* sorted_gid, const uint32_t* tile_order, const AttrRecord* rec, uint32_t width,
                 uint32_t height, const uint8_t* mask, const float* values, uint32_t channels, double* out, double* out_weight,
                 hipStream_t s);

}
```

3dgs.cpp_amd/csrc/gs_preprocess.hip:

```cpp
#include "gs_bin.h"

namespace gs {

constexpr float SH_C0 = 0.28209479177387814f;
constexpr float SH_C1 = 0.4886025119029199f;

__device__ __forceinline__ float ndc2pix(float v, int S) { return ((v + 1.0f) * (float)S - 1.0f) * 0.5f; }

struct PreUniforms {
    gs_uniforms u;
    Counters* counters;
    const FrameParams* fp;
    uint64_t* stamps;
};

template <int R1>
struct PreBins {
    uint32_t tbl[R1 ? 64 * R1 : 1];
    uint32_t vis;
};

constexpr int kPrePlane = 68, kPreStage = 4 * kPrePlane + 16;
constexpr int kPreShHalf = 32;
constexpr int kPreWaveLds = kPreShHalf * 12 + 4;
static_assert(kPreWaveLds >= kPreStage, "the record stage must fit the wave's LDS slab");

template <class SH>
__device__ __forceinline__ void sh_to_rgb(const SH& S, float x, float y, float z, float (&rgb)[3]) {
    const float C2_0 = 1.0925484305920792f, C2_1 = -1.0925484305920792f, C2_2 = 0.31539156525252005f,
                C2_3 = -1.0925484305920792f, C2_4 = 0.5462742152960396f;
    const float C3_0 = -0.5900435899266435f, C3_1 = 2.890611442640554f, C3_2 = -0.4570457994644658f,
                C3_3 = 0.3731763325901154f, C3_4 = -0.4570457994644658f, C3_5 = 1.445305721320277f,
                C3_6 = -0.5900435899266435f;
    float c[3];
#define GS_SH_FENCE() asm volatile("" : "+v"(c[0]), "+v"(c[1]), "+v"(c[2]) :: "memory")
#pragma unroll
    for (int k = 0; k < 3; ++k) c[k] = SH_C0 * S(0, k);
#pragma unroll
    for (int k = 0; k < 3; ++k) c[k] -= SH_C1 * S(1, k) * y;
#pragma unroll
    for (int k = 0; k < 3; ++k) c[k] += SH_C1 * S(2, k) * z;
#pragma unroll
    for (int k = 0; k < 3; ++k) c[k] -= SH_C1 * S(3, k) * x;
    GS_SH_FENCE();
#pragma unroll
    for (int k = 0; k < 3; ++k) c[k] += C2_0 * S(4, k) * x * y;
#pragma unroll
    for (int k = 0; k < 3; ++k) c[k] += C2_1 * S(5, k) * y * z;
#pragma unroll
    for (int k = 0; k < 3; ++k) c[k] += C2_2 * S(6, k) * (2.0f * z * z - x * x - y * y);
#pragma unroll
    for (int k = 0; k < 3; ++k) c[k] += C2_3 * S(7, k) * z * x;
    GS_SH_FENCE();
#pragma unroll
    for (int k = 0; k < 3; ++k) c[k] += C2_4 * S(8, k) * (x * x - y * y);
#pragma unroll
    for (int k = 0; k < 3; ++k) c[k] += C3_0 * S(9, k) * (3.0f * x * x - y * y) * y;
#pragma unroll
    for (int k = 0; k < 3; ++k) c[k] += C3_1 * S(10, k) * x * y * z;
#pragma unroll
    for (int k = 0; k < 3; ++k) c[k] += C3_2 * S(11, k) * (4.0f * z * z - x * x - y * y) * y;
    GS_SH_FENCE();
#pragma unroll
    for (int k = 0; k < 3; ++k) c[k] += C3_3 * S(12, k) * z * (2.0f * z * z - 3.0f * x * x - 3.0f * y * y);
#pragma unroll
    for (int k = 0; k < 3; ++k) c[k] += C3_4 * S(13, k) * x * (4.0f * z * z - x * x - y * y);
#pragma unroll
    for (int k = 0; k < 3; ++k) c[k] += C3_5 * S(14, k) * (x * x - y * y) * z;
#pragma unroll
    for (int k = 0; k < 3; ++k) c[k] += C3_6 * S(15, k) * x * (x * x - 3.0f * y * y);
#pragma unroll
    for (int k = 0; k < 3; ++k) rgb[k] = c[k] + 0.5f;
#undef GS_SH_FENCE
    if (rgb[0] < 0.0f) rgb[0] = 0.0f;
}
struct ShFromLds {
    const float* p;
    __device__ __forceinline__ float operator()(int j, int k) const { return p[j * 3 + k]; }
};
struct ShFromLds16 {
    const uint16_t* p;
    __device__ __forceinline__ float operator()(int j, int k) const { return __half2float(__ushort_as_half(p[j * 3 + k])); }
};
// ... 140 lines not shown
        {
            const uint32_t x0 = bb & 255u, y0 = (bb >> 8) & 255u, x1 = (bb >> 16) & 255u, y1 = bb >> 24;
            const bool big = (x1 - x0) * (y1 - y0) > kL1BigBox;
            if (!big)
                for (uint32_t y = y0; y < y1; ++y)
                    for (uint32_t x = x0; x < x1; ++x) atomicAdd(&bins.tbl[(y << lf.grid_shift) | x], 1u);
            for (uint64_t bm = __ballot(big); bm != 0; bm &= bm - 1) {
                const uint32_t b1 = (uint32_t)__builtin_amdgcn_readlane((int)bb, __ffsll((unsigned long long)bm) - 1);
                const uint32_t gx0 = b1 & 255u, gy0 = (b1 >> 8) & 255u, bw = ((b1 >> 16) & 255u) - gx0, cells = bw * ((b1 >> 24) - gy0);
                for (uint32_t c = lane; c < cells; c += WAVE) atomicAdd(&bins.tbl[((gy0 + c / bw) << lf.grid_shift) | (gx0 + c % bw)], 1u);
            }
            const uint32_t nv = (uint32_t)__popcll(__ballot(vis));
            if (lane == 0 && nv) atomicAdd(&bins.vis, nv);
        }
        __syncthreads();
#pragma unroll
        for (int k = 0; k < NB / BLOCK; ++k) {
            const uint32_t b = (uint32_t)(k * BLOCK + tid), cnt = bins.tbl[b];
            fbase[k] = cnt ? atomicAdd(lf.words + (size_t)(kL1FusedCursor0 + b) * kL1FusedStride, cnt) : 0u;
        }
        if (tid == 0 && bins.vis)
            __hip_atomic_fetch_add(lf.words + (size_t)((i / BLOCK) % kVisRegions) * kL1FusedStride, bins.vis, __ATOMIC_RELAXED, __HIP_MEMORY_SCOPE_AGENT);
    }

    float rgb[3] = {0.0f, 0.0f, 0.0f};
    const uint64_t vm_sh = __ballot(vis);
    const uint32_t n_vis = (uint32_t)__popcll(vm_sh);
    const uint32_t my_rank = (uint32_t)__popcll(vm_sh & ((1ull << lane) - 1ull));
    uint8_t* const s_src = reinterpret_cast<uint8_t*>(stage + kPreShHalf * 12);
    if (vis) s_src[my_rank] = (uint8_t)lane;
    __builtin_amdgcn_wave_barrier();
    const int chunks = sv.sh16 ? 6 : 12;
    const uint32_t per_inst = sv.sh16 ? 10u : 5u;
    const uint32_t slot = sv.sh16 ? lane / 6u : lane / 12u, q = sv.sh16 ? lane % 6u : lane % 12u;
    const char* const sh_bytes = sv.sh16 ? reinterpret_cast<const char*>(sv.sh16) : reinterpret_cast<const char*>(blob + (size_t)P_SH * N);
    const size_t sh_stride = sv.sh16 ? 96 : 192;
    const uint32_t lds_base = (uint32_t)__builtin_amdgcn_readfirstlane((int)(uint32_t)(uintptr_t)stage);
    for (uint32_t half = 0; half * kPreShHalf < n_vis; ++half) {
        const uint32_t first = half * kPreShHalf, last = min(n_vis, first + (uint32_t)kPreShHalf);
        uint32_t dst = lds_base;
        for (uint32_t g0 = first; g0 < last; g0 += per_inst, dst += per_inst * (uint32_t)sh_stride) {
            const uint32_t g = g0 + slot;
            if (lane < 60u && g < last) {
                const uint32_t src_lane = s_src[g];
                const char* gsrc = sh_bytes + (size_t)(i - lane + src_lane) * sh_stride + q * 16u;
                unsigned keep;
                asm volatile("s_mov_b32 %0, m0\n\ts_mov_b32 m0, %2\n\ts_nop 0\n\tglobal_load_lds_dwordx4 %1, off\n\ts_mov_b32 m0, %0"
                             : "=&s"(keep) : "v"(gsrc), "s"(dst) : "memory");
            }
        }
        asm volatile("s_waitcnt vmcnt(0)" ::: "memory");
        __builtin_amdgcn_wave_barrier();
        if (vis && my_rank >= first && my_rank < last) {
            float dx = px - u.camera_position[0];
            float dy = py - u.camera_position[1];
            float dz = pz - u.camera_position[2];
            const float len = sqrtf(dx * dx + dy * dy + dz * dz);
            const float x = dx / len, y = dy / len, z = dz / len;
            const float4* blk = stage + (size_t)(my_rank - first) * chunks;
            if (sv.sh16) {
                sh_to_rgb(ShFromLds16{reinterpret_cast<const uint16_t*>(blk)}, x, y, z, rgb);
            } else {
                sh_to_rgb(ShFromLds{reinterpret_cast<const float*>(blk)}, x, y, z, rgb);
            }
            if (!av.vis && R1 == 0) {
                av.depth[oid] = depth;
                av.aabb[oid] = make_ushort4((unsigned short)bx0, (unsigned short)by0, (unsigned short)bx1, (unsigned short)by1);
            }
        }
        __builtin_amdgcn_wave_barrier();
    }
    if (R1 == 0 && valid && !av.vis) av.tiles[oid] = num_tiles;
    if constexpr (R1 != 0) {
        const uint64_t m = __ballot(vis);
        if (lane == 0 && valid) lf.vis_mask[i / WAVE] = m;
    }

    if constexpr (R1 != 0) {
        constexpr int NB = 64 * R1;
#pragma unroll
        for (int k = 0; k < NB / BLOCK; ++k) bins.tbl[k * BLOCK + (int)threadIdx.x] = fbase[k];
        __syncthreads();
        const BinGrid g{lf.tiles_x, lf.tiles_y, lf.bins_x, lf.bins_y, lf.bin_shift, lf.grid_shift};
        auto emit = [&](uint32_t bin, uint32_t k, uint32_t gid, ushort4 box) {
            const uint32_t pos = atomicAdd(&bins.tbl[bin], 1u);
            if (pos < lf.cap) {
                const uint32_t sb = (bin >> lf.grid_shift) * lf.bins_x + (bin & ((1u << lf.grid_shift) - 1u));
                uint32_t* const rec = lf.cand + (size_t)kCandWords * ((size_t)sb * lf.cap + pos);
                rec[0] = k;
                rec[1] = gid;
                rec[2] = bin_local_box16(g, bin, box);
            }
        };
        const uint32_t x0 = bb & 255u, y0 = (bb >> 8) & 255u, x1 = (bb >> 16) & 255u, y1 = bb >> 24;
        const ushort4 tb = make_ushort4((unsigned short)bx0, (unsigned short)by0, (unsigned short)bx1, (unsigned short)by1);
        const uint32_t key = __float_as_uint(depth);
        const bool big = (x1 - x0) * (y1 - y0) > kL1BigBox;
        if (!big)
            for (uint32_t y = y0; y < y1; ++y)
                for (uint32_t x = x0; x < x1; ++x) emit((y << lf.grid_shift) | x, key, oid, tb);
        for (uint64_t bm = __ballot(big); bm != 0; bm &= bm - 1) {
            const int src = __ffsll((unsigned long long)bm) - 1;
            const uint32_t b1 = (uint32_t)__builtin_amdgcn_readlane((int)bb, src);
            const uint32_t gx0 = b1 & 255u, gy0 = (b1 >> 8) & 255u, bw = ((b1 >> 16) & 255u) - gx0, cells = bw * ((b1 >> 24) - gy0);
            const uint32_t bkey = (uint32_t)__builtin_amdgcn_readlane((int)key, src), bgid = (uint32_t)__builtin_amdgcn_readlane((int)oid, src);
            const uint32_t blo = (uint32_t)__builtin_amdgcn_readlane((int)((uint32_t)bx0 | ((uint32_t)by0 << 16)), src);
            const uint32_t bhi = (uint32_t)__builtin_amdgcn_readlane((int)((uint32_t)bx1 | ((uint32_t)by1 << 16)), src);
            const ushort4 bbox = make_ushort4((unsigned short)(blo & 0xFFFFu), (unsigned short)(blo >> 16), (unsigned short)(bhi & 0xFFFFu),
                                              (unsigned short)(bhi >> 16));
            for (uint32_t c = lane; c < cells; c += WAVE) emit(((gy0 + c / bw) << lf.grid_shift) | (gx0 + c % bw), bkey, bgid, bbox);
        }
    }

    const uint64_t vm = __ballot(vis);
    if (av.vis) {
        const uint32_t base = (uint32_t)__builtin_amdgcn_readfirstlane((int)vis_base);
        if (vis)
            av.vis[base + (uint32_t)__popcll(vm & ((1ull << lane) - 1ull))] =
                make_uint4(oid, __float_as_uint(depth), (uint32_t)bx0 | ((uint32_t)by0 << 16), (uint32_t)bx1 | ((uint32_t)by1 << 16));
    }
    if (vis) {
        stage[0 * kPrePlane + lane] = make_float4(c00, c01, c11, opacity);
        stage[1 * kPrePlane + lane] = make_float4(uvx, uvy, rgb[0], rgb[1]);
        const float r11 = -c01 * __builtin_amdgcn_rcpf(c11), r00 = -c01 * __builtin_amdgcn_rcpf(c00);
        stage[2 * kPrePlane + lane] = make_float4(rgb[2], acut, r11, r00);
        stage[3 * kPrePlane + lane] = make_float4(depth, radii, 0.0f, 0.0f);
    }
    uint32_t* const s_oid = reinterpret_cast<uint32_t*>(stage + 4 * kPrePlane);
    if (sv.perm) s_oid[lane] = oid;
    __builtin_amdgcn_wave_barrier();
    {
        float4* const rec0 = reinterpret_cast<float4*>(av.rec + (i - lane));
        const uint32_t c = lane & 3u;
#pragma unroll
        for (int t = 0; t < 4; ++t) {
            const uint32_t r = (uint32_t)t * 16u + (lane >> 2);
            if ((vm >> r) & 1ull) {
                const float4 val = stage[c * kPrePlane + r];
                float4* const dst = sv.perm ? reinterpret_cast<float4*>(av.rec + s_oid[r]) + c : rec0 + (size_t)r * 4 + c;
                *dst = val;
            }
        }
    }
}

template <bool AA, int R1>
__global__ __launch_bounds__(BLOCK) void k_preprocess(SceneView sv, PreUniforms pu, AttrView av, L1Fused lf) {
    __shared__ float4 s_stage[BLOCK / WAVE][kPreWaveLds];
    __shared__ PreBins<R1> s_bins;
    if constexpr (R1 != 0) {
        for (int b = threadIdx.x; b < 64 * R1; b += BLOCK) s_bins.tbl[b] = 0;
        if (threadIdx.x == 0) s_bins.vis = 0;
    }
    const gs_uniforms& u = pu.fp ? pu.fp->u : pu.u;
    const uint32_t i = blockIdx.x * BLOCK + threadIdx.x;
    frame_stamp(pu.stamps, ST_PREPROCESS);
    if (i == 0 && pu.counters) {
        pu.counters->visible = 0;
        pu.counters->instances = 0;
        pu.counters->overflow = 0;
        pu.counters->bin_entries = 0;
        pu.counters->max_bin = 0;
        pu.counters->slabs = 0;
        pu.counters->blend_resolved = 0;
        pu.counters->blend_redo = 0;
        pu.counters->q_head = 0;
        pu.counters->q_bins_done = 0;
    }
    preprocess_one<AA, R1>(sv, u, av, i, i < sv.n, s_stage[threadIdx.x / WAVE], lf, s_bins);
}

__global__ __launch_bounds__(BLOCK) void k_records_to_planes(const uint64_t* __restrict__ vis_mask, const uint32_t* __restrict__ perm,
                                                             const AttrRecord* __restrict__ rec, uint32_t n, uint32_t width, uint32_t height,
                                                             uint32_t* __restrict__ tiles, float* __restrict__ depth, ushort4* __restrict__ aabb) {
    const uint32_t j = blockIdx.x * BLOCK + threadIdx.x;
    if (j >= n) return;
    const uint32_t oid = perm ? perm[j] : j;
    uint32_t nt = 0;
    if ((vis_mask[j / WAVE] >> (j % WAVE)) & 1ull) {
        const AttrRecord r = rec[oid];
        const int tile_w = (int)((width + kTile - 1) / kTile), tile_h = (int)((height + kTile - 1) / kTile);
        const float uvx = r.uv_rg.x, uvy = r.uv_rg.y, radii = r.depth_radius.y;
        const int bx0 = clampi(f2i_sat((uvx - radii) / kTile), 0, tile_w);
        const int by0 = clampi(f2i_sat((uvy - radii) / kTile), 0, tile_h);
        const int bx1 = clampi(f2i_sat((uvx + radii + kTile - 1) / kTile), 0, tile_w);
        const int by1 = clampi(f2i_sat((uvy + radii + kTile - 1) / kTile), 0, tile_h);
        nt = (uint32_t)(bx1 - bx0) * (uint32_t)(by1 - by0);
        depth[oid] = r.depth_radius.x;
        aabb[oid] = make_ushort4((unsigned short)bx0, (unsigned short)by0, (unsigned short)bx1, (unsigned short)by1);
    }
    tiles[oid] = nt;
}
void launch_records_to_planes(const uint64_t* vis_mask, const uint32_t* perm, const AttrView& av, uint32_t n, uint32_t width, uint32_t height,
                              hipStream_t s) {
    if (n == 0) return;
    hipLaunchKernelGGL(k_records_to_planes, dim3((n + BLOCK - 1) / BLOCK), dim3(BLOCK), 0, s, vis_mask, perm, av.rec, n, width, height, av.tiles,
                       av.depth, av.aabb);
}

void launch_preprocess(const SceneView& sv, const gs_uniforms& u, const AttrView& av, Counters* counters,
                       const FrameParams* fp, uint64_t* stamps, bool antialiased, const L1Fused& lf, hipStream_t s) {
    if (sv.n == 0) return;
    PreUniforms pu;
    pu.u = u;
    pu.counters = counters;
    pu.fp = fp;
    pu.stamps = stamps;
    const dim3 grid((sv.n + BLOCK - 1) / BLOCK);
    const int r1 = !lf.words ? 0 : (lf.grid_shift == 4 ? 4 : 16);
#define GS_PRE_CASE(A, R)                                                                       \
    if (antialiased == A && r1 == R) {                                                          \
        hipLaunchKernelGGL((k_preprocess<A, R>), grid, dim3(BLOCK), 0, s, sv, pu, av, lf);      \
        return;                                                                                 \
    }
    GS_PRE_CASE(false, 0)
    GS_PRE_CASE(false, 4)
    GS_PRE_CASE(false, 16)
    GS_PRE_CASE(true, 0)
    GS_PRE_CASE(true, 4)
    GS_PRE_CASE(true, 16)
#undef GS_PRE_CASE
}
}
```

3dgs.cpp_amd/csrc/gs_renderer.cpp:

```cpp
#include <algorithm>
#include <chrono>
#include <cstdio>
#include <cstdlib>
#include <cstring>
#include <limits>
#include <memory>
#include <vector>

#include "gs_blend_tuner.h"
#include "gs_depth_policy.h"
#include "gs_internal.h"

using namespace gs_host;

struct FrameBuffers {
    hipStream_t stream = nullptr;
    DevBuf<uint32_t> tiles;
    DevBuf<float> depth;
    DevBuf<ushort4> aabb;
    DevBuf<gs::AttrRecord> rec;
    DevBuf<uint4> vis;
    DevBuf<uint32_t> vis_count;
    int planes_stale = 0;
    DevBuf<uint64_t> vis_mask;
    uint32_t vis_region_slots = 0;
    DevBuf<uint32_t> dkeys[2], dvals[2];
    DevBuf<uint32_t> block_hist, digit_total;
    DevBuf<uint32_t> l1_hist, bin_count;
    DevBuf<uint32_t> cand;
    DevBuf<uint32_t> l1_words;
    DevBuf<uint32_t> sorted;
    DevBuf<uint32_t> ranges;
    DevBuf<uint8_t> slabs;
    uint32_t slab_epoch = 0;
    DevBuf<gs::Counters> counters;
    DevBuf<uint64_t> stamps;
    DevBuf<gs::FrameParams> params;
    hipGraphExec_t graph_execs[2] = {nullptr, nullptr};
    struct GraphKey {
        int level = -1, bin_shift = -1, hw_exp = 0, contract = 1;
        bool antialiased = false, lockstep = false, l1_fused = false;
        uint32_t width = 0, height = 0, capacity = 0, cand_capacity = 0;
        const void *tile_order = nullptr, *ranges = nullptr, *sh16 = nullptr;
        bool operator==(const GraphKey& o) const {
            return level == o.level && bin_shift == o.bin_shift && hw_exp == o.hw_exp && contract == o.contract &&
                   antialiased == o.antialiased && lockstep == o.lockstep && l1_fused == o.l1_fused &&
                   width == o.width && height == o.height && capacity == o.capacity && cand_capacity == o.cand_capacity &&
                   tile_order == o.tile_order && ranges == o.ranges && sh16 == o.sh16;
        }
    } graph_keys[2];
    void drop_graph(int which) {
        if (graph_execs[which]) (void)hipGraphExecDestroy(graph_execs[which]);
        graph_execs[which] = nullptr;
        graph_keys[which] = GraphKey{};
    }
    void drop_graph() {
        drop_graph(0);
        drop_graph(1);
    }
    size_t n = 0;
    bool ready = false;

    void init(size_t n_, uint32_t capacity, uint32_t cand_capacity, bool dense_lists) {
        n = n_;
        HIP_CHECK(hipStreamCreateWithFlags(&stream, hipStreamNonBlocking));
        tiles.alloc(n);
        depth.alloc(n);
        aabb.alloc(n);
        rec.alloc(n);
        vis_region_slots = gs::vis_region_slots(static_cast<uint32_t>(n));
        if (dense_lists) ensure_dense_lists();
        l1_hist.alloc(1025 * static_cast<size_t>(gs::bin_level1_columns(static_cast<uint32_t>(n))));
        bin_count.alloc(2048);
        vis_mask.alloc((n + 63) / 64 + 1);
        l1_words.alloc(gs::kL1FusedWords);
        HIP_CHECK(hipMemset(l1_words.p, 0, l1_words.n * sizeof(uint32_t)));
        counters.alloc(1);
        stamps.alloc(gs::ST_COUNT);
        HIP_CHECK(hipMemset(stamps.p, 0, gs::ST_COUNT * sizeof(uint64_t)));
        params.alloc(1);
        set_capacity(capacity);
        set_cand_capacity(cand_capacity);
        ready = true;
    }
    void ensure_dense_lists() {
        if (vis.p) return;
        vis.alloc(static_cast<size_t>(gs::kVisRegions) * vis_region_slots);
        vis_count.alloc(gs::kVisRegions * gs::kVisCounterStride);
        HIP_CHECK(hipMemset(vis_count.p, 0, vis_count.n * sizeof(uint32_t)));
    }
    void ensure_depth_order() {
        if (dkeys[0].p) return;
        for (int k = 0; k < 2; ++k) {
            dkeys[k].alloc(n);
            dvals[k].alloc(n);
        }
        block_hist.alloc(256 * static_cast<size_t>(gs::kSortMaxBlocks));
        digit_total.alloc(256);
    }
    void set_capacity(uint32_t cap) {
        drop_graph();
        sorted.alloc(static_cast<size_t>(cap) + 4);
    }
    void set_cand_capacity(uint32_t ccap) {
        drop_graph();
        cand.alloc(3 * static_cast<size_t>(ccap));
        HIP_CHECK(hipMemset(cand.p, 0, 3 * static_cast<size_t>(ccap) * sizeof(uint32_t)));
    }
    void sync() const { HIP_CHECK(hipStreamSynchronize(stream)); }
    void sync_nothrow() const { (void)hipStreamSynchronize(stream); }
    ~FrameBuffers() {
        drop_graph();
        if (stream) (void)hipStreamDestroy(stream);
    }
};

struct FrameSlot {
    gs_uniforms u{};
    float* rgba = nullptr;
    uint8_t* bgra = nullptr;
    hipEvent_t done = nullptr;
    gs::Counters* h_counters = nullptr;
    uint64_t* h_stamps = nullptr;
    gs::FrameParams* h_params = nullptr;
    bool timed = false;
    int level = 0;
    int bin_shift = 3;
    bool lockstep = false;
    bool l1_fused = false;
    uint32_t l1_cap = 0;
    uint32_t tune_round = 0;
    int tune_shape = 0;
};

struct gs_renderer {
    static constexpr int kMaxInFlight = 8;
    static constexpr int kSlots = 2 * kMaxInFlight;

    gs_scene* scene = nullptr;
    bool timing = true;
    double tick_ms = 1e-5;

    FrameBuffers sets[kMaxInFlight];
    int num_sets = 1;
    uint32_t capacity = 0;
    uint32_t cand_capacity = 0;
    uint32_t default_cand_capacity = 0;
    L1FusedPolicy l1_policy;
    bool last_l1_fused = false;
    FrameBuffers* last_set = nullptr;
    uint32_t last_width = 0, last_height = 0;

    FrameSlot slots[kSlots];
    int in_flight_limit = 1;
    uint64_t frames_enqueued = 0;
    int pending = 0;

    gs_frame_stats last{};

    DepthPolicy policy;
    static constexpr int kGlobalLevel = DepthPolicy::kGlobalLevel;
    bool graph_mode = false;
    int exp_mode = 3;
    int blend_exp_mode() const { return exp_mode == 3 && !contract && !scene->unit_opacity ? 2 : exp_mode; }
    bool contract = false;
    bool antialiased = false;
    BlendTunerBank tuners;
    uint64_t dense_min = 4u << 20;
    bool dense_for_spatial = std::getenv("GS_L1_DENSE_MIN") == nullptr;
    bool wants_dense_lists() const { return scene->n >= dense_min || (dense_for_spatial && scene->perm.p); }
    bool debug_levels = std::getenv("GS_DEBUG_LEVELS") != nullptr;
    bool level2_queue = !(std::getenv("GS_L2_QUEUE") && std::atoi(std::getenv("GS_L2_QUEUE")) == 0);
    double stall_ms = std::getenv("GS_DEBUG_STALLS") ? std::atof(std::getenv("GS_DEBUG_STALLS")) : 0.0;
    static constexpr int kLaps = 10;
    std::chrono::steady_clock::time_point laps[kLaps];
    void lap(int k) {
        if (stall_ms > 0.0) laps[k] = std::chrono::steady_clock::now();
    }
    void report_stall() {
        if (stall_ms <= 0.0) return;
        auto ms = [&](int a, int b) { return std::chrono::duration<double, std::milli>(laps[b] - laps[a]).count(); };
        if (ms(0, 9) < stall_ms) return;
        std::fprintf(stderr, "[gs3d] stall: frame %llu held the host %.3f ms: wait-for-slot %.3f, setup %.3f, preprocess %.3f, order %.3f, level1 %.3f, "
                             "level2 %.3f, blend %.3f, closing events %.3f\n", (unsigned long long)(frames_enqueued - 1), ms(0, 9), ms(0, 1), ms(1, 2), ms(2, 3),
                     ms(3, 4), ms(4, 5), ms(5, 6), ms(6, 7), ms(7, 9));
    }
    bool have_frame = false;
    uint32_t retries = 0;
    uint32_t redo_chain = 0;
    double total_ms[7] = {0, 0, 0, 0, 0, 0, 0};
    uint64_t total_frames = 0;
    uint64_t lifetime_frames = 0;
    static constexpr size_t kIntervalRing = 8192;
    std::vector<float> intervals;
    bool prev_retired = false;
    uint64_t latest_done = 0;

    uint32_t* sorted_gid = nullptr;
    uint32_t* depth_order = nullptr;
    uint64_t num_tiles = 0;

    ~gs_renderer() {
        for (auto& sl : slots) {
            if (sl.done) (void)hipEventDestroy(sl.done);
            if (sl.h_counters) (void)hipHostFree(sl.h_counters);
            if (sl.h_stamps) (void)hipHostFree(sl.h_stamps);
            if (sl.h_params) (void)hipHostFree(sl.h_params);
        }
    }

    void set_capacity(uint32_t cap) {
        capacity = cap;
        for (auto& fb : sets)
            if (fb.ready) fb.set_capacity(cap);
    }
    void set_cand_capacity(uint32_t ccap) {
        cand_capacity = ccap;
        for (auto& fb : sets)
            if (fb.ready) fb.set_cand_capacity(ccap);
    }

    void init() {
        if (const char* e = std::getenv("GS_BLEND_LOCKSTEP")) tuners.pin(std::atoi(e) < 0 ? -1 : (std::atoi(e) != 0 ? 1 : 0));
        HIP_CHECK(hipSetDevice(scene->device));
        {
            int khz = 0;
            if (hipDeviceGetAttribute(&khz, hipDeviceAttributeWallClockRate, scene->device) == hipSuccess && khz > 0) tick_ms = 1.0 / khz;
        }
        HIP_CHECK(gs::bin_prepare_device());
        if (std::getenv("GS_DEBUG_OCCUPANCY")) gs::bin_debug_occupancy();
        for (auto& sl : slots) {
            HIP_CHECK(hipEventCreateWithFlags(&sl.done, hipEventDisableTiming));
            HIP_CHECK(hipHostMalloc(reinterpret_cast<void**>(&sl.h_stamps), gs::ST_COUNT * sizeof(uint64_t), hipHostMallocDefault));
            std::memset(sl.h_stamps, 0, gs::ST_COUNT * sizeof(uint64_t));
            HIP_CHECK(hipHostMalloc(reinterpret_cast<void**>(&sl.h_counters), sizeof(gs::Counters), hipHostMallocDefault));
            *sl.h_counters = gs::Counters{};
            HIP_CHECK(hipHostMalloc(reinterpret_cast<void**>(&sl.h_params), sizeof(gs::FrameParams), hipHostMallocDefault));
        }
        uint64_t want = std::max<uint64_t>(1u << 20, 8 * static_cast<uint64_t>(scene->n));
        if (const char* e = std::getenv("GS_INITIAL_CAPACITY")) want = std::max<uint64_t>(256, std::strtoull(e, nullptr, 10));
        capacity = static_cast<uint32_t>(std::min<uint64_t>(want, kMaxInstances));
        uint64_t want_cand = std::max<uint64_t>(1u << 18, 2 * static_cast<uint64_t>(scene->n));
        if (const char* e = std::getenv("GS_INITIAL_CAND_CAPACITY")) want_cand = std::max<uint64_t>(256, std::strtoull(e, nullptr, 10));
        else if (std::getenv("GS_INITIAL_CAPACITY")) want_cand = std::min<uint64_t>(want_cand, want);
        cand_capacity = static_cast<uint32_t>(std::min<uint64_t>(want_cand, capacity));
        default_cand_capacity = cand_capacity;
        sets[0].init(scene->n, capacity, cand_capacity, wants_dense_lists());
    }

    void set_num_sets(int k) {
        for (int i = 0; i < k; ++i)
            if (!sets[i].ready) sets[i].init(scene->n, capacity, cand_capacity, wants_dense_lists());
        num_sets = k;
    }

    DevBuf<uint32_t> tile_order;
    uint32_t order_tx = 0, order_ty = 0;
    void ensure_tile_order(uint32_t tx, uint32_t ty) {
        if (tx == order_tx && ty == order_ty && tile_order.p) return;
        drain();
        constexpr uint32_t B = 4;
        const uint64_t nt = static_cast<uint64_t>(tx) * ty;
        std::vector<std::vector<uint32_t>> per_xcd(8);
        const uint32_t nbx = (tx + B - 1) / B, nby = (ty + B - 1) / B;
        for (uint32_t by = 0; by < nby; ++by)
            for (uint32_t bx = 0; bx < nbx; ++bx) {
                auto& list = per_xcd[(bx + 3 * by) % 8];
                for (uint32_t y = by * B; y < std::min(ty, (by + 1) * B); ++y)
                    for (uint32_t x = bx * B; x < std::min(tx, (bx + 1) * B); ++x) list.push_back(y * tx + x);
            }
        std::vector<uint32_t> order(nt);
        size_t cursor[8] = {0, 0, 0, 0, 0, 0, 0, 0};
        for (uint64_t b = 0; b < nt; ++b) {
            int x = static_cast<int>(b % 8);
            if (cursor[x] >= per_xcd[x].size()) {
                size_t best = 0;
                for (int k = 0; k < 8; ++k)
                    if (per_xcd[k].size() - cursor[k] > best) best = per_xcd[k].size() - cursor[k], x = k;
            }
            order[b] = per_xcd[x][cursor[x]++];
        }
        tile_order.ensure(nt);
        if (nt) HIP_CHECK(hipMemcpy(tile_order.p, order.data(), nt * sizeof(uint32_t), hipMemcpyHostToDevice));
        order_tx = tx;
        order_ty = ty;
    }

    BinGeometry bin_geometry(uint32_t tx, uint32_t ty) const {
        BinGeometry g;
        if (!policy.bin_geometry(tx, ty, &g)) throw Error(GS_ERR_INVALID, "resolution too large for the tile binning (max 16384 x 16384)");
        return g;
    }

    void validate(const gs_uniforms& u) const {
        const uint32_t tx = tiles_across(u.width), ty = tiles_across(u.height);
        if (tx > 65535 || ty > 65535) throw Error(GS_ERR_INVALID, "resolution too large (tile box is 16-bit)");
        (void)bin_geometry(tx, ty);
    }

    void forget_last_frame() {
        have_frame = false;
        last_set = nullptr;
        last_width = last_height = 0;
        num_tiles = 0;
        sorted_gid = depth_order = nullptr;
    }
    bool has_last_frame() const { return have_frame && last_set != nullptr; }

    bool lacks_buffers(const FrameBuffers& fb, uint64_t nt, int lv) const {
        return 2 * nt > fb.ranges.n || (lv >= kGlobalLevel && !fb.dkeys[0].p) || (lv == gs::kBinSlabLevel && !fb.slabs.p);
    }
    L1FusedPolicy::Verdict l1_verdict(const gs_uniforms& u) const {
        const BinGeometry g = bin_geometry(tiles_across(u.width), tiles_across(u.height));
        return l1_policy.decide(policy.frame_level() < kGlobalLevel && g.bin_shift <= 3, scene->n < dense_min, scene->perm.p != nullptr,
                                u.width, u.height, g.bin_shift, cand_capacity, g.bins_x * g.bins_y);
    }
    uint32_t l1_growth(const gs_uniforms& u) const {
        if (scene->n == 0 || u.width == 0 || u.height == 0) return 0;
        const BinGeometry g = bin_geometry(tiles_across(u.width), tiles_across(u.height));
        return l1_policy.grow_to(l1_verdict(u), u.width, u.height, g.bin_shift, cand_capacity, g.bins_x * g.bins_y, default_cand_capacity);
    }

    void enqueue(const gs_uniforms& u, float* d_rgba, uint8_t* d_bgra) {
        validate(u);
        HIP_CHECK(hipSetDevice(scene->device));
        const uint32_t tx = tiles_across(u.width), ty = tiles_across(u.height);
        const bool new_grid = !(tx == order_tx && ty == order_ty && tile_order.p);
        if (pending > 0 && (new_grid || lacks_buffers(sets[frames_enqueued % num_sets], static_cast<uint64_t>(tx) * ty, policy.frame_level()) ||
                            l1_growth(u) != 0))
            drain();
        try {
            issue(u, d_rgba, d_bgra);
        } catch (...) {
            forget_last_frame();
            throw;
        }
    }

    void issue(const gs_uniforms& u, float* d_rgba, uint8_t* d_bgra) {
        FrameSlot& sl = slots[frames_enqueued % kSlots];
        FrameBuffers& fb = sets[frames_enqueued % num_sets];
        hipStream_t stream = fb.stream;
        const uint32_t n = static_cast<uint32_t>(scene->n);
        const uint32_t tx = tiles_across(u.width), ty = tiles_across(u.height);
        const uint64_t nt = static_cast<uint64_t>(tx) * ty;
        const bool fused_counters = n != 0 && u.width != 0 && u.height != 0;
        const int lv = policy.frame_level();
        if (lacks_buffers(fb, nt, lv)) {
            fb.ranges.ensure(2 * nt);
            if (lv >= kGlobalLevel) fb.ensure_depth_order();
            if (lv == gs::kBinSlabLevel && !fb.slabs.p) {
                fb.slabs.alloc(static_cast<size_t>(gs::kSlabCapacity) * gs::kSlabDescBytes);
                HIP_CHECK(hipMemset(fb.slabs.p, 0, fb.slabs.n));
            }
        }
        if (const uint32_t grow = l1_growth(u); grow > cand_capacity) set_cand_capacity(grow);
        ensure_tile_order(tx, ty);
        const int tune_shape = tuners.select(u.width, u.height);
        const BlendTuner& tuner = tuners.current();
        const bool lockstep = tuner.current();
        const BinGeometry geo = bin_geometry(tx, ty);
        const bool bin_local = lv < kGlobalLevel;
        lap(2);

        gs::SceneView sv{scene->render_blob(), scene->cov3d.p, n, static_cast<uint32_t>(gs::blob_stride(n)),
                          scene->sh_half ? scene->sh16.p : nullptr, scene->acut.p, scene->perm.p};
        gs::Counters* cnt = fb.counters.p;
        const bool l1_any_order = bin_local && geo.bin_shift <= 3;
        const bool l1_fused = fused_counters && l1_verdict(u) == L1FusedPolicy::kEngage;
        const bool dense_list = l1_any_order && !l1_fused && n != 0 && wants_dense_lists() && fb.vis.p && u.width != 0 && u.height != 0;
        gs::AttrView av{fb.tiles.p, fb.depth.p, fb.aabb.p, fb.rec.p, dense_list ? fb.vis.p : nullptr, dense_list ? fb.vis_count.p : nullptr,
                        fb.vis_region_slots};
        const uint32_t l1_cap = L1FusedPolicy::region_cap(cand_capacity, geo.bins_x * geo.bins_y);
        const gs::L1Fused lf{l1_fused ? fb.l1_words.p : nullptr, fb.cand.p, l1_cap, fb.vis_mask.p, tx, ty, geo.bins_x, geo.bins_y, geo.bin_shift, geo.grid_shift};
        fb.planes_stale = dense_list ? 1 : (l1_fused ? 2 : 0);

        if (!fused_counters) {
            HIP_CHECK(hipMemsetAsync(cnt, 0, sizeof(gs::Counters), stream));
            HIP_CHECK(hipMemsetAsync(fb.ranges.p, 0, 2 * nt * sizeof(uint32_t), stream));
        }
        uint64_t* const stamps = fb.stamps.p;
        auto passes = [&](const gs::FrameParams* fp) {
            gs::launch_preprocess(sv, u, av, cnt, fp, stamps, antialiased, lf, stream);
            lap(3);
            if (!bin_local && n != 0) {
                const int blocks = std::max(1, std::min<int>(gs::kSortMaxBlocks, (n + gs::kSortTileKeys - 1) / gs::kSortTileKeys));
                const uint32_t* kin = reinterpret_cast<const uint32_t*>(fb.depth.p);
                const uint32_t* vin = nullptr;
                for (int pass = 0; pass < 4; ++pass) {
                    gs::RadixPass p{};
                    const int dst = pass & 1;
                    p.keys_in = kin;
                    p.vals_in = vin;
                    p.keys_out = fb.dkeys[dst].p;
                    p.vals_out = fb.dvals[dst].p;
                    p.n_in = &cnt->visible;
                    p.n_static = n;
                    p.tiles = fb.tiles.p;
                    p.n_out = &cnt->visible;
                    p.block_hist = fb.block_hist.p;
                    p.digit_total = fb.digit_total.p;
                    p.shift = pass * 8;
                    p.bits = 8;
                    p.blocks = blocks;
                    p.first = pass == 0;
                    p.stamps = pass == 0 ? stamps : nullptr;
                    gs::launch_radix_pass(p, stream);
                    kin = fb.dkeys[dst].p;
                    vin = fb.dvals[dst].p;
                }
            }
            lap(4);
            if (n != 0) {
                gs::BinLaunch b{};
                b.order = bin_local ? nullptr : fb.dvals[1].p;
                b.n_items = bin_local ? nullptr : &cnt->visible;
                b.n_bound = n;
                b.tiles = fb.tiles.p;
                b.aabb = fb.aabb.p;
                b.depth = fb.depth.p;
                b.vis = av.vis;
                b.vis_count = av.vis_count;
                b.vis_region_slots = av.vis_region_slots;
                b.hist = fb.l1_hist.p;
                b.bin_count = fb.bin_count.p;
                b.cand = fb.cand.p;
                b.ranges = fb.ranges.p;
                b.sorted_gid = fb.sorted.p;
                b.counters = cnt;
                b.capacity = capacity;
                b.cand_capacity = cand_capacity;
                b.l1_fused_words = lf.words;
                b.l1_fused_cap = l1_cap;
                b.slabs = fb.slabs.p;
                b.slab_capacity = fb.slabs.p ? gs::kSlabCapacity : 0u;
                b.slab_epoch = 0;
                if (level2_queue && !fp && lv == gs::kBinSlabLevel) {
                    if (++fb.slab_epoch == 0) ++fb.slab_epoch;
                    b.slab_epoch = fb.slab_epoch;
                }
                b.tiles_x = tx;
                b.tiles_y = ty;
                b.bins_x = geo.bins_x;
                b.bins_y = geo.bins_y;
                b.bin_shift = geo.bin_shift;
                b.grid_shift = geo.grid_shift;
                b.stamps = stamps;
                if (!l1_fused) {
                    gs::launch_bin_level1_count(b, stream);
                    gs::launch_bin_level1_scatter(b, l1_any_order, stream);
                }
                lap(5);
                gs::launch_bin_level2(b, lv, stream);
            }
            lap(6);
            gs::launch_blend(fb.ranges.p, fb.sorted.p, tile_order.p, av, u.width, u.height, d_rgba, d_bgra, cnt,
                             fused_counters ? sl.h_counters : nullptr, blend_exp_mode(), contract, fp, lockstep, stamps, stream);
            gs::launch_frame_end(stamps, sl.h_stamps, fp, lf.words, gs::kVisRegions + (1u << (2 * geo.grid_shift)), stream);
            lap(7);
        };
        const bool replay = graph_mode && fused_counters;
        if (replay) {
            *sl.h_params = gs::FrameParams{u, d_rgba, d_bgra, sl.h_counters, sl.h_stamps};
            HIP_CHECK(hipMemcpyAsync(fb.params.p, sl.h_params, sizeof(gs::FrameParams), hipMemcpyHostToDevice, stream));
            const FrameBuffers::GraphKey key{lv, geo.bin_shift, blend_exp_mode(), contract ? 1 : 0,
                                             antialiased, lockstep, l1_fused,
                                             u.width, u.height, capacity, cand_capacity,
                                             tile_order.p, fb.ranges.p, sv.sh16};
            const int gi = lockstep ? 1 : 0;
            if (!fb.graph_execs[gi] || !(key == fb.graph_keys[gi])) {
                fb.drop_graph(gi);
                hipGraph_t graph = nullptr;
                HIP_CHECK(hipStreamBeginCapture(stream, hipStreamCaptureModeThreadLocal));
                try {
                    passes(fb.params.p);
                } catch (...) {
                    (void)hipStreamEndCapture(stream, &graph);
                    if (graph) (void)hipGraphDestroy(graph);
                    throw;
                }
                HIP_CHECK(hipStreamEndCapture(stream, &graph));
                const hipError_t e = hipGraphInstantiate(&fb.graph_execs[gi], graph, nullptr, nullptr, 0);
                (void)hipGraphDestroy(graph);
                HIP_CHECK(e);
                fb.graph_keys[gi] = key;
            }
            HIP_CHECK(hipGraphLaunch(fb.graph_execs[gi], stream));
        } else {
            passes(nullptr);
        }
        if (!fused_counters) HIP_CHECK(hipMemcpyAsync(sl.h_counters, cnt, sizeof(gs::Counters), hipMemcpyDeviceToHost, stream));
        HIP_CHECK(hipEventRecord(sl.done, stream));
        HIP_CHECK(hipGetLastError());

        last_set = &fb;
        last_width = u.width;
        last_height = u.height;
        num_tiles = nt;
        last_l1_fused = l1_fused;
        depth_order = bin_local ? nullptr : fb.dvals[1].p;
        sorted_gid = fb.sorted.p;

        sl.level = lv;
        sl.bin_shift = geo.bin_shift;
        sl.lockstep = lockstep;
        sl.l1_fused = l1_fused;
        sl.l1_cap = l1_cap;
        sl.tune_round = tuner.round;
        sl.tune_shape = tune_shape;
        sl.u = u;
        sl.rgba = d_rgba;
        sl.bgra = d_bgra;
        sl.timed = fused_counters;
        ++frames_enqueued;
        ++pending;
        lap(9);
    }

    FrameSlot& oldest() { return slots[(frames_enqueued - pending) % kSlots]; }
    FrameSlot& queued(int k) { return slots[(frames_enqueued - pending + k) % kSlots]; }

    void retire_oldest() {
        FrameSlot& sl = oldest();
        HIP_CHECK(hipEventSynchronize(sl.done));
        if (sl.h_counters->overflow) {
            rerun_queued();
            return;
        }
        redo_chain = 0;
        policy.frame_retired(sl.level, sl.h_counters->max_bin, sl.bin_shift);
        l1_policy.frame_retired(sl.u.width, sl.u.height, sl.bin_shift, sl.h_counters->max_bin, sl.h_counters->bin_entries, sl.h_counters->visible);
        last = frame_stats(sl);
        have_frame = true;
        const float v[7] = {last.ms_preprocess, last.ms_prefix_sum, last.ms_preprocess_sort, last.ms_sort,
                            last.ms_tile_boundary, last.ms_render, last.ms_total};
        for (int k = 0; k < 7; ++k) total_ms[k] += v[k];
        ++total_frames;
        ++lifetime_frames;
        note_completion(sl, last.ms_total);
        --pending;
    }

    void rerun_queued() {
        for (auto& fb : sets)
            if (fb.ready) fb.sync();
        struct Redo {
            gs_uniforms u;
            float* rgba;
            uint8_t* bgra;
        };
        std::vector<Redo> redo;
        std::vector<DepthPolicy::QueuedFrame> ran;
        uint64_t need = 0, need_cand = 0;
        for (int k = 0; k < pending; ++k) {
            const FrameSlot& q = queued(k);
            const gs::Counters& c = *q.h_counters;
            redo.push_back({q.u, q.rgba, q.bgra});
            ran.push_back({q.level, q.bin_shift, q.u.width, q.u.height, c.overflow, c.max_bin});
            if (q.l1_fused && (c.overflow & 1u) && c.max_bin > q.l1_cap) l1_policy.region_overflowed();
            if (c.overflow & 1u) {
                if (c.bin_entries > cand_capacity) need_cand = std::max<uint64_t>(need_cand, c.bin_entries);
                else need = std::max<uint64_t>(need, c.instances);
            }
        }
        if (debug_levels) report_overflow();
        frames_enqueued -= pending;
        pending = 0;
        prev_retired = false;
        forget_last_frame();
        switch (policy.frames_overflowed(ran.data(), static_cast<int>(ran.size()))) {
            case DepthPolicy::kDepthsTooCrowded:
                throw Error(GS_ERR_OVERFLOW, "a bin's depths are too crowded for the bin-local order (one depth bucket beyond a slab, or more than 65 equal depths in one): needs the global depth-order path");
            case DepthPolicy::kBinTooFull:
                throw Error(GS_ERR_OVERFLOW, "a bin holds more candidates than the bin-local sort can order");
            case DepthPolicy::kRerun:
                break;
        }
        if (++redo_chain > 8) throw Error(GS_ERR_OVERFLOW, "instance buffers overflowed repeatedly");
        if (need_cand > cand_capacity) {
            need_cand = need_cand + need_cand / 2 + 4096;
            if (need_cand > kMaxInstances) throw Error(GS_ERR_OVERFLOW, "more than 2^30 level-1 candidates");
            set_cand_capacity(static_cast<uint32_t>(need_cand));
        }
        if (need > capacity) {
            need = need + need / 2 + 4096;
            if (need > kMaxInstances) throw Error(GS_ERR_OVERFLOW, "more than 2^30 tile instances");
            set_capacity(static_cast<uint32_t>(need));
        }
        ++retries;
        for (const Redo& f : redo) enqueue(f.u, f.rgba, f.bgra);
    }

    void report_overflow() {
        std::fprintf(stderr, "[gs3d] frame %llu overflowed at level %d (refined %d, hold %u):", (unsigned long long)(frames_enqueued - pending),
                     oldest().level, (int)policy.refined, policy.slab_hold);
        for (int k = 0; k < pending; ++k) {
            const FrameSlot& q = queued(k);
            std::fprintf(stderr, " [lvl %d bin 2^%d ovf %u max_bin %u E1 %u D %u slabs %u]", q.level, q.bin_shift, q.h_counters->overflow,
                         q.h_counters->max_bin, q.h_counters->bin_entries, q.h_counters->instances, q.h_counters->slabs);
        }
        std::fprintf(stderr, " capacity %u candidates %u\n", capacity, cand_capacity);
    }

    gs_frame_stats frame_stats(const FrameSlot& sl) const {
        gs_frame_stats st{};
        st.num_gaussians = scene->n;
        st.num_visible = sl.h_counters->visible;
        st.num_instances = sl.h_counters->instances;
        st.num_bin_entries = sl.h_counters->bin_entries;
        st.max_bin_entries = sl.h_counters->max_bin;
        st.sort_path = sl.level < kGlobalLevel ? 2u : 1u;
        st.sort_level = static_cast<uint32_t>(sl.level);
        st.bin_tiles = 1u << sl.bin_shift;
        st.instance_capacity = capacity;
        const uint64_t* const ts = sl.h_stamps;
// ... 213 lines not shown

int gs_set_sort_path(gs_renderer* r, int mode) {
    return guarded([&] {
        if (!r) throw Error(GS_ERR_INVALID, "renderer is null");
        if (mode < 0 || mode > 2) throw Error(GS_ERR_INVALID, "sort path must be 0 (auto), 1 (global) or 2 (bin-local)");
        r->drain();
        r->policy.set_sort_mode(mode);
    });
}

int gs_set_exp_mode(gs_renderer* r, int mode) {
    return guarded([&] {
        if (!r) throw Error(GS_ERR_INVALID, "renderer is null");
        if (mode < 0 || mode > 3)
            throw Error(GS_ERR_INVALID, "exp mode must be 0 (pipeline polynomial), 1 (hardware v_exp_f32), 2 (libm's expf in binary64) or 3 (guarded v_exp_f32)");
        r->drain();
        r->exp_mode = mode;
    });
}

int gs_set_blend_contraction(gs_renderer* r, int enabled) {
    return guarded([&] {
        if (!r) throw Error(GS_ERR_INVALID, "renderer is null");
        r->drain();
        r->contract = enabled != 0;
    });
}

int gs_set_antialiased(gs_renderer* r, int enabled) {
    return guarded([&] {
        if (!r) throw Error(GS_ERR_INVALID, "renderer is null");
        r->drain();
        r->antialiased = enabled != 0;
    });
}

int gs_get_antialiased(gs_renderer* r) {
    int on = 0;
    const int rc = guarded([&] {
        if (!r) throw Error(GS_ERR_INVALID, "renderer is null");
        on = r->antialiased ? 1 : 0;
    });
    return rc != 0 ? rc : on;
}

int gs_set_blend_lockstep(gs_renderer* r, int mode) {
    return guarded([&] {
        if (!r) throw Error(GS_ERR_INVALID, "null argument");
        if (mode < -1 || mode > 1) throw Error(GS_ERR_INVALID, "blend lockstep: -1 automatic, 0 off, 1 on");
        r->drain();
        r->tuners.pin(mode);
    });
}

int gs_get_blend_lockstep(gs_renderer* r, int* settled) {
    int now = 0;
    const int rc = guarded([&] {
        if (!r) throw Error(GS_ERR_INVALID, "null argument");
        const BlendTuner& t = r->tuners.current();
        now = t.current() ? 1 : 0;
        if (settled) *settled = (t.forced >= 0 || t.phase == 3) ? 1 : 0;
    });
    return rc != 0 ? rc : now;
}

int gs_set_level1_fused(gs_renderer* r, int mode) {
    return guarded([&] {
        if (!r) throw Error(GS_ERR_INVALID, "null argument");
        if (mode < -1 || mode > 1) throw Error(GS_ERR_INVALID, "level-1 fusion: -1 by rule, 0 off, 1 on");
        r->drain();
        r->l1_policy.mode = mode;
    });
}

int gs_get_level1_fused(gs_renderer* r) {
    int on = 0;
    const int rc = guarded([&] {
        if (!r) throw Error(GS_ERR_INVALID, "null argument");
        on = r->last_l1_fused ? 1 : 0;
    });
    return rc != 0 ? rc : on;
}

int gs_set_graph_mode(gs_renderer* r, int enabled) {
    return guarded([&] {
        if (!r) throw Error(GS_ERR_INVALID, "renderer is null");
        r->drain();
        r->graph_mode = enabled != 0;
        if (!r->graph_mode)
            for (auto& fb : r->sets) fb.drop_graph();
    });
}

int gs_debug_download(gs_renderer* r, int stage, void* dst, uint64_t bytes) {
    return guarded([&] {
        if (!r || !dst) throw Error(GS_ERR_INVALID, "null argument");
        r->drain();
        if (!r->has_last_frame()) throw Error(GS_ERR_INVALID, "no frame rendered yet");
        if (stage == GS_STAGE_DEPTH_ORDER && !r->depth_order)
            throw Error(GS_ERR_INVALID, "the depth-order tap exists only on the global depth-order path (gs_set_sort_path(r, 1))");
        const uint64_t n = r->scene->n, v = r->last.num_visible;
        const uint64_t d = std::min<uint64_t>(r->last.num_instances, r->capacity);
        const void* src = nullptr;
        uint64_t size = 0;
        if (r->last_set->planes_stale && (stage == GS_STAGE_TILES || stage == GS_STAGE_DEPTH || stage == GS_STAGE_AABB)) {
            FrameBuffers& fb = *r->last_set;
            const gs::AttrView pv{fb.tiles.p, fb.depth.p, fb.aabb.p, fb.rec.p, fb.vis.p, fb.vis_count.p, fb.vis_region_slots};
            if (fb.planes_stale == 1) gs::launch_vis_to_planes(pv, static_cast<uint32_t>(n), fb.stream);
            else gs::launch_records_to_planes(fb.vis_mask.p, r->scene->perm.p, pv, static_cast<uint32_t>(n), r->last_width, r->last_height, fb.stream);
            HIP_CHECK(hipGetLastError());
            HIP_CHECK(hipStreamSynchronize(fb.stream));
            fb.planes_stale = 0;
        }
        switch (stage) {
            case GS_STAGE_TILES: src = r->last_set->tiles.p; size = n * 4; break;
            case GS_STAGE_DEPTH: src = r->last_set->depth.p; size = n * 4; break;
            case GS_STAGE_RADIUS:
            case GS_STAGE_CONIC_OPACITY:
            case GS_STAGE_UV_RG:
            case GS_STAGE_B:
            case GS_STAGE_ALPHA_CUT:
                {
                    const size_t width = stage == GS_STAGE_RADIUS || stage == GS_STAGE_B || stage == GS_STAGE_ALPHA_CUT ? 1 : 4;
                    if (bytes < n * width * 4) throw Error(GS_ERR_INVALID, "destination too small for stage buffer");
                    std::vector<gs::AttrRecord> recs(n);
                    if (n) HIP_CHECK(hipMemcpy(recs.data(), r->last_set->rec.p, n * sizeof(gs::AttrRecord), hipMemcpyDeviceToHost));
                    float* out = static_cast<float*>(dst);
                    for (uint64_t i = 0; i < n; ++i) {
                        const gs::AttrRecord& a = recs[i];
                        if (stage == GS_STAGE_RADIUS) out[i] = a.depth_radius.y;
                        else if (stage == GS_STAGE_B) out[i] = a.b_cut_r.x;
                        else if (stage == GS_STAGE_ALPHA_CUT) out[i] = a.b_cut_r.y;
                        else std::memcpy(out + 4 * i, stage == GS_STAGE_CONIC_OPACITY ? &a.conic_op : &a.uv_rg, 16);
                    }
                    return;
                }
            case GS_STAGE_AABB: src = r->last_set->aabb.p; size = n * 8; break;
            case GS_STAGE_DEPTH_ORDER: src = r->depth_order; size = v * 4; break;
            case GS_STAGE_SORTED_TILE:
            case GS_STAGE_SORTED_GID:
            case GS_STAGE_RANGES:
                {
                    const uint64_t nt = r->num_tiles;
                    std::vector<uint32_t> rg(2 * nt);
                    if (nt) HIP_CHECK(hipMemcpy(rg.data(), r->last_set->ranges.p, rg.size() * 4, hipMemcpyDeviceToHost));
                    if (stage == GS_STAGE_RANGES) {
                        if (bytes < nt * 8) throw Error(GS_ERR_INVALID, "destination too small for stage buffer");
                        uint32_t* out = static_cast<uint32_t*>(dst);
                        uint64_t pos = 0;
                        for (uint64_t t = 0; t < nt; ++t) {
                            const uint32_t len = rg[2 * t + 1] - rg[2 * t];
                            out[2 * t] = len ? static_cast<uint32_t>(pos) : 0u;
                            out[2 * t + 1] = len ? static_cast<uint32_t>(pos + len) : 0u;
                            pos += len;
                        }
                        return;
                    }
                    if (bytes < d * 4) throw Error(GS_ERR_INVALID, "destination too small for stage buffer");
                    std::vector<uint32_t> lists;
                    if (stage == GS_STAGE_SORTED_GID) {
                        lists.resize(r->capacity);
                        HIP_CHECK(hipMemcpy(lists.data(), r->sorted_gid, lists.size() * 4, hipMemcpyDeviceToHost));
                    }
                    uint32_t* out = static_cast<uint32_t*>(dst);
                    uint64_t pos = 0;
                    for (uint64_t t = 0; t < nt; ++t)
                        for (uint64_t i = rg[2 * t]; i < rg[2 * t + 1] && pos < d; ++i)
                            out[pos++] = stage == GS_STAGE_SORTED_GID ? lists[i] : static_cast<uint32_t>(t);
                    return;
                }
            case GS_STAGE_LISTS_RAW: src = r->sorted_gid; size = d * 4; break;
            case GS_STAGE_RANGES_RAW: src = r->last_set->ranges.p; size = r->num_tiles * 8; break;
            default: throw Error(GS_ERR_INVALID, "unknown stage");
        }
        if (bytes < size) throw Error(GS_ERR_INVALID, "destination too small for stage buffer");
        if (size) HIP_CHECK(hipMemcpy(dst, src, size, hipMemcpyDeviceToHost));
    });
}

int gs_accumulate_contributions(gs_renderer* r, const gs_contributions* c) {
    return guarded([&] {
        if (!r || !c) throw Error(GS_ERR_INVALID, "null argument");
        if (reinterpret_cast<uintptr_t>(c->weight) % 8 != 0) throw Error(GS_ERR_INVALID, "weight must be 8-byte aligned");
        if (reinterpret_cast<uintptr_t>(c->pixels) % 4 != 0) throw Error(GS_ERR_INVALID, "pixels must be 4-byte aligned");
        if (reinterpret_cast<uintptr_t>(c->top_id) % 4 != 0) throw Error(GS_ERR_INVALID, "top_id must be 4-byte aligned");
        r->over_last_frame(!c->weight && !c->pixels && !c->top_id, [&](const FrameBuffers& fb) {
            gs::launch_contributions(fb.ranges.p, fb.sorted.p, r->tile_order.p, fb.rec.p, r->last_width, r->last_height, c->mask,
                                     c->weight, c->pixels, c->top_id, fb.stream);
        });
    });
}

int gs_blend_features(gs_renderer* r, const gs_feature_maps* m) {
    return guarded([&] {
        if (!r || !m) throw Error(GS_ERR_INVALID, "null argument");
        if (m->channels > GS_FEATURE_CHANNELS_MAX) throw Error(GS_ERR_INVALID, "channels exceeds GS_FEATURE_CHANNELS_MAX (256)");
        if (m->channels > 0 && !m->features) throw Error(GS_ERR_INVALID, "channels > 0 needs features");
        if (m->channels > 0 && !m->out_features) throw Error(GS_ERR_INVALID, "features given without out_features");
        const struct { const void* p; const char* what; } ptrs[] = {
            {m->features, "features must be 4-byte aligned"},         {m->out_features, "out_features must be 4-byte aligned"},
            {m->out_alpha, "out_alpha must be 4-byte aligned"},       {m->out_depth, "out_depth must be 4-byte aligned"},
            {m->out_depth_median, "out_depth_median must be 4-byte aligned"}};
        for (const auto& q : ptrs)
            if (reinterpret_cast<uintptr_t>(q.p) % 4 != 0) throw Error(GS_ERR_INVALID, q.what);
        float* out_features = m->channels > 0 ? m->out_features : nullptr;
        r->over_last_frame(!out_features && !m->out_alpha && !m->out_depth && !m->out_depth_median, [&](const FrameBuffers& fb) {
            gs::launch_features(fb.ranges.p, fb.sorted.p, r->tile_order.p, fb.rec.p, r->last_width, r->last_height, m->features,
                                m->channels, out_features, m->out_alpha, m->out_depth, m->out_depth_median, fb.stream);
        });
    });
}

int gs_lift_pixels(gs_renderer* r, const gs_pixel_lift* l) {
    return guarded([&] {
        if (!r || !l) throw Error(GS_ERR_INVALID, "null argument");
        if (l->channels > GS_LIFT_CHANNELS_MAX) throw Error(GS_ERR_INVALID, "channels exceeds GS_LIFT_CHANNELS_MAX (256)");
        if (l->channels > 0 && !l->values) throw Error(GS_ERR_INVALID, "channels > 0 needs values");
        if (l->channels > 0 && !l->out) throw Error(GS_ERR_INVALID, "values given without out");
        if (reinterpret_cast<uintptr_t>(l->values) % 4 != 0) throw Error(GS_ERR_INVALID, "values must be 4-byte aligned");
        if (reinterpret_cast<uintptr_t>(l->out) % 8 != 0) throw Error(GS_ERR_INVALID, "out must be 8-byte aligned");
        if (reinterpret_cast<uintptr_t>(l->out_weight) % 8 != 0) throw Error(GS_ERR_INVALID, "out_weight must be 8-byte aligned");
        double* out = l->channels > 0 ? l->out : nullptr;
        r->over_last_frame(!out && !l->out_weight, [&](const FrameBuffers& fb) {
            gs::launch_lift(fb.ranges.p, fb.sorted.p, r->tile_order.p, fb.rec.p, r->last_width, r->last_height, l->mask, l->values,
                            l->channels, out, l->out_weight, fb.stream);
        });
    });
}

void* gs_renderer_stream(gs_renderer* r) { return r ? r->sets[0].stream : nullptr; }

}
```

include/gs3d_hip.h:

```cpp
#ifndef GS3D_HIP_H
#define GS3D_HIP_H

#include <stdint.h>

#ifdef __cplusplus
extern "C" {
#endif

typedef struct gs_scene gs_scene;
typedef struct gs_renderer gs_renderer;

enum gs_status {
    GS_OK = 0,
    GS_ERR_INVALID = -1,
    GS_ERR_IO = -2,
    GS_ERR_DEVICE = -3,
    GS_ERR_NOMEM = -4,
    GS_ERR_OVERFLOW = -5
};

typedef struct {
    float position[3];
    float rotation[4];
    float fov;
    float near_plane;
    float far_plane;
} gs_camera;

typedef struct {
    float camera_position[4];
    float proj_mat[16];
    float view_mat[16];
    uint32_t width;
    uint32_t height;
    float tan_fovx;
    float tan_fovy;
} gs_uniforms;

typedef struct {
    uint64_t num_gaussians;
    uint64_t num_visible;
    uint64_t num_instances;
    uint64_t instance_capacity;
    float ms_preprocess;
    float ms_prefix_sum;
    float ms_preprocess_sort;
    float ms_sort;
    float ms_tile_boundary;
    float ms_render;
    float ms_total;
    uint32_t retries;
    uint32_t num_bin_entries;
    uint32_t max_bin_entries;
    uint32_t sort_path;
    uint32_t bin_tiles;
    uint32_t sort_level;
    uint32_t blend_redo;
    uint32_t blend_resolved;
    uint32_t pad_;
} gs_frame_stats;

enum gs_stage {
    GS_STAGE_TILES = 0,
    GS_STAGE_DEPTH = 1,
    GS_STAGE_RADIUS = 2,
    GS_STAGE_AABB = 3,
    GS_STAGE_CONIC_OPACITY = 4,
    GS_STAGE_UV_RG = 5,
    GS_STAGE_B = 6,
    GS_STAGE_DEPTH_ORDER = 7,
    GS_STAGE_ALPHA_CUT = 8,
    GS_STAGE_SORTED_TILE = 11,
    GS_STAGE_SORTED_GID = 12,
    GS_STAGE_RANGES = 13,
    GS_STAGE_LISTS_RAW = 14,
    GS_STAGE_RANGES_RAW = 15
};

const char* gs_last_error(void);
int gs_device_count(int* count);


int gs_scene_load_ply(const char* path, int device, gs_scene** out);

int gs_read_ply(const char* path, float* records, uint64_t capacity, uint64_t* n_out);
int gs_activate_records(const float* records, uint64_t n, float* vertices);

int gs_scene_from_records(const float* records, uint64_t n, int device, gs_scene** out);

int gs_scene_from_vertices(const float* vertices, uint64_t n, int device, gs_scene** out);

int gs_scene_from_device_blob(float* d_blob, uint64_t n, int device, gs_scene** out);
uint64_t gs_scene_blob_floats(uint64_t n);
int gs_scene_blob(const gs_scene* s, float** d_blob, uint64_t* floats);

typedef struct {
    const float* means;
    const float* log_scales;
    const float* quats;
    const float* opacity_logits;
    const float* sh_dc;
    const float* sh_rest;
    uint32_t     sh_rest_coeffs;
} gs_device_arrays;

int gs_scene_from_device_arrays(const gs_device_arrays* a, uint64_t n, int device, void* stream, gs_scene** out);
int gs_scene_update_from_device_arrays(gs_scene* s, const gs_device_arrays* a, uint64_t first, uint64_t count, void* stream);

typedef struct {
    float rotation[4];
    float translation[3];
    float scale;
} gs_transform;
int gs_scene_transform(gs_scene* s, const gs_transform* t, uint64_t first, uint64_t count, void* stream);
int gs_transform_sh_matrices(const gs_transform* t, float out[83]);
int gs_transform_camera(const gs_transform* t, const gs_camera* in, gs_camera* out);

int gs_deactivate_vertices(const float* vertices, uint64_t n, float* records);
int gs_write_ply(const char* path, const float* records, uint64_t n);
typedef struct {
    float* means;
    float* log_scales;
    float* quats;
    float* opacity_logits;
    float* sh_dc;
    float* sh_rest;
    uint32_t sh_rest_coeffs;
} gs_device_arrays_out;
int gs_scene_to_device_arrays(const gs_scene* s, const gs_device_arrays_out* a, uint64_t first, uint64_t count, void* stream);
int gs_scene_download_records(const gs_scene* s, uint64_t first, uint64_t count, float* records);
int gs_scene_save_ply(const gs_scene* s, const char* path);

uint64_t gs_scene_num_vertices(const gs_scene* s);
int gs_scene_quantize_sh(gs_scene* s);
int gs_scene_sh_bits(const gs_scene* s);
int gs_scene_download_vertex_range(const gs_scene* s, uint64_t first, uint64_t count, float* vertices);
int gs_scene_download_vertices(const gs_scene* s, float* vertices);
int gs_scene_download_cov3d(const gs_scene* s, float* cov3d);
void gs_scene_destroy(gs_scene* s);


int gs_renderer_create(gs_scene* scene, gs_renderer** out);
void gs_renderer_destroy(gs_renderer* r);

int gs_camera_uniforms(const gs_camera* cam, uint32_t width, uint32_t height, gs_uniforms* out);

int gs_render(gs_renderer* r, const gs_uniforms* u, float* d_rgba, uint8_t* d_bgra);

int gs_render_host(gs_renderer* r, const gs_uniforms* u, float* h_rgba, uint8_t* h_bgra);

int gs_synchronize(gs_renderer* r);
int gs_set_timing(gs_renderer* r, int enabled);
int gs_set_frames_in_flight(gs_renderer* r, int frames);
int gs_set_sort_path(gs_renderer* r, int mode);
int gs_set_exp_mode(gs_renderer* r, int mode);
int gs_set_blend_contraction(gs_renderer* r, int enabled);
int gs_set_antialiased(gs_renderer* r, int enabled);
int gs_get_antialiased(gs_renderer* r);
int gs_set_graph_mode(gs_renderer* r, int enabled);
int gs_set_blend_lockstep(gs_renderer* r, int mode);
int gs_get_blend_lockstep(gs_renderer* r, int* settled);
int gs_set_level1_fused(gs_renderer* r, int mode);
int gs_get_level1_fused(gs_renderer* r);
int gs_get_timing_totals(gs_renderer* r, gs_frame_stats* sum, uint64_t* frames, int reset);
int gs_get_frame_intervals(gs_renderer* r, float* out_ms, uint64_t capacity, uint64_t* n_out, int reset);
int gs_get_stats(gs_renderer* r, gs_frame_stats* out);
int gs_poll_stats(gs_renderer* r, gs_frame_stats* out, uint64_t* frames_retired);
int gs_debug_download(gs_renderer* r, int stage, void* dst, uint64_t bytes);
typedef struct {
    const uint8_t* mask;
    uint64_t* weight;
    uint32_t* pixels;
    uint32_t* top_id;
} gs_contributions;
int gs_accumulate_contributions(gs_renderer* r, const gs_contributions* c);
#define GS_FEATURE_CHANNELS_MAX 256
typedef struct {
    const float* features;
    uint32_t     channels;
    float* out_features;
    float* out_alpha;
    float* out_depth;
    float* out_depth_median;
} gs_feature_maps;
int gs_blend_features(gs_renderer* r, const gs_feature_maps* m);
#define GS_LIFT_CHANNELS_MAX 256
typedef struct {
    const float*   values;
    uint32_t       channels;
    const uint8_t* mask;
    double*        out;
    double*        out_weight;
} gs_pixel_lift;
int gs_lift_pixels(gs_renderer* r, const gs_pixel_lift* l);
int gs_debug_expf_scan(int device, uint32_t first_bits, uint64_t count, uint64_t* block_sums, uint64_t blocks_capacity, double* guard);
int gs_debug_activation_expf_scan(int device, uint32_t first_bits, uint64_t count, uint64_t* block_sums, uint64_t blocks_capacity);
int gs_debug_alpha_cut_scan(int device, uint32_t first_bits, uint64_t count, uint64_t* mismatches, uint32_t* first_mismatch);
void* gs_renderer_stream(gs_renderer* r);

#define GS_DIST_ID_BYTES 128
typedef struct gs_dist gs_dist;
int gs_dist_unique_id(uint8_t id[GS_DIST_ID_BYTES]);
int gs_dist_create(const uint8_t id[GS_DIST_ID_BYTES], int rank, int world, int device, gs_dist** out);
int gs_dist_rank(const gs_dist* d);
int gs_dist_world(const gs_dist* d);
uint64_t gs_dist_pose_count(const gs_dist* d, uint64_t poses);
int gs_dist_broadcast_scene(gs_dist* d, gs_scene* mine , int root, gs_scene** out);
#define GS_DIST_COPY_ON_ROOT 1u
int gs_dist_broadcast_scene_ex(gs_dist* d, gs_scene* mine , int root, unsigned flags, gs_scene** out);
typedef struct {
    uint64_t ranks;
    uint64_t world;
    uint64_t checksum;
    uint64_t broadcast_bytes;
    double broadcast_ms;
    uint32_t checksums_equal;
    uint32_t rccl_version;
} gs_dist_report;
int gs_dist_verify(gs_dist* d, const gs_scene* scene, gs_dist_report* out);
void gs_dist_destroy(gs_dist* d);

#ifdef __cplusplus
}
#endif
#endif
```

Baseline: 5272.

## Cull per-tile Gaussian instances with tight ellipse-vs-alpha-cut tile bounds

Preprocess now computes a conservative tight tile box per Gaussian from its conic and alpha cutoff and packs it next to the reference box in the candidate record. The level-2 bin builder (fused L1 path) emits only the tiles inside the tight box, which shrinks the per-tile lists the blender walks. It still counts reference instances for capacity and debug parity, and adds a second atomic counter plus extra record loads. The feature is on by default (GS_TILE_CULL env to disable) and is part of the graph key.

```diff
diff --git a/3dgs.cpp_amd/binding.py b/3dgs.cpp_amd/binding.py
--- a/3dgs.cpp_amd/binding.py
+++ b/3dgs.cpp_amd/binding.py
@@ -15,7 +15,7 @@
 BLOB_PLANES = 59
 
 
-KERNEL_SOURCES = ("gs_device.h", "gs_bin.h", "gs_scene.hip", "gs_preprocess.hip", "gs_radix.hip", "gs_bin_l1.hip", "gs_bin_l2.hip",
+KERNEL_SOURCES = ("gs_device.h", "gs_bin.h", "gs_tile_cull.h", "gs_scene.hip", "gs_preprocess.hip", "gs_radix.hip", "gs_bin_l1.hip", "gs_bin_l2.hip",
                   "gs_blend.hip", "gs_contrib.hip", "gs_features.hip", "gs_lift.hip", "gs_kernels.h")
 
 
@@ -38,7 +38,8 @@
 STAGES = dict(tiles=(0, np.uint32), depth=(1, np.float32), radius=(2, np.float32), aabb=(3, np.uint16),
               conic_opacity=(4, np.float32), uv_rg=(5, np.float32), b=(6, np.float32),
               depth_order=(7, np.uint32), alpha_cut=(8, np.float32), sorted_tile=(11, np.uint32), sorted_gid=(12, np.uint32),
-              ranges=(13, np.uint32), lists_raw=(14, np.uint32), ranges_raw=(15, np.uint32))
+              ranges=(13, np.uint32), lists_raw=(14, np.uint32), ranges_raw=(15, np.uint32),
+              lists_culled=(16, np.uint32), ranges_culled=(17, np.uint32))
 
 SYMBOLS = ["gs_last_error", "gs_device_count", "gs_read_ply", "gs_activate_records", "gs_scene_load_ply", "gs_scene_from_records",
            "gs_scene_from_vertices", "gs_scene_from_device_blob", "gs_scene_blob_floats", "gs_scene_blob",
@@ -48,7 +49,7 @@
            "gs_scene_download_vertices", "gs_scene_download_cov3d",
            "gs_deactivate_vertices", "gs_write_ply", "gs_scene_to_device_arrays", "gs_scene_download_records", "gs_scene_save_ply",
            "gs_scene_destroy", "gs_renderer_create", "gs_renderer_destroy", "gs_camera_uniforms",
-           "gs_render", "gs_render_host", "gs_synchronize", "gs_set_timing", "gs_set_frames_in_flight", "gs_set_sort_path", "gs_set_exp_mode", "gs_set_graph_mode", "gs_set_blend_lockstep", "gs_get_blend_lockstep", "gs_set_level1_fused", "gs_get_level1_fused", "gs_set_blend_contraction", "gs_set_antialiased", "gs_get_antialiased", "gs_get_timing_totals",
+           "gs_render", "gs_render_host", "gs_synchronize", "gs_set_timing", "gs_set_frames_in_flight", "gs_set_sort_path", "gs_set_exp_mode", "gs_set_graph_mode", "gs_set_blend_lockstep", "gs_get_blend_lockstep", "gs_set_level1_fused", "gs_get_level1_fused", "gs_set_tile_cull", "gs_get_tile_cull", "gs_get_listed_instances", "gs_set_blend_contraction", "gs_set_antialiased", "gs_get_antialiased", "gs_get_timing_totals",
            "gs_get_frame_intervals", "gs_get_stats", "gs_poll_stats", "gs_debug_download", "gs_accumulate_contributions", "gs_blend_features", "gs_lift_pixels", "gs_debug_expf_scan", "gs_debug_alpha_cut_scan", "gs_renderer_stream",
            "gs_dist_unique_id", "gs_dist_create", "gs_dist_rank", "gs_dist_world", "gs_dist_pose_count",
            "gs_dist_broadcast_scene", "gs_dist_broadcast_scene_ex", "gs_dist_verify", "gs_dist_destroy"]
@@ -632,6 +633,21 @@
             _check(now)
         return bool(now)
 
+    def set_tile_cull(self, on):
+        _check(lib().gs_set_tile_cull(self._h, C.c_int(1 if on else 0)))
+
+    def tile_cull(self):
+        culled = C.c_int(0)
+        now = lib().gs_get_tile_cull(self._h, C.byref(culled))
+        if now < 0:
+            _check(now)
+        return bool(now), bool(culled.value)
+
+    def listed_instances(self):
+        out = C.c_uint64(0)
+        _check(lib().gs_get_listed_instances(self._h, C.byref(out)))
+        return int(out.value)
+
     def set_sort_path(self, mode):
         _check(lib().gs_set_sort_path(self._h, C.c_int(int(mode))))
 
@@ -664,7 +680,9 @@
         n, v, d = st.num_gaussians, st.num_visible, min(st.num_instances, st.instance_capacity)
         count = {"tiles": n, "depth": n, "radius": n, "aabb": 4 * n, "conic_opacity": 4 * n, "uv_rg": 4 * n,
                  "b": n, "alpha_cut": n, "depth_order": v, "sorted_tile": d, "sorted_gid": d, "lists_raw": d}.get(name)
-        if name in ("ranges", "ranges_raw"):
+        if name == "lists_culled":
+            count = min(self.listed_instances(), st.instance_capacity)
+        if name in ("ranges", "ranges_raw", "ranges_culled"):
             w, h = int(uniforms["width"][0]), int(uniforms["height"][0])
             count = 2 * ((w + 15) // 16) * ((h + 15) // 16)
         out = np.zeros(max(int(count), 1), dt)
diff --git a/3dgs.cpp_amd/csrc/gs_bin.h b/3dgs.cpp_amd/csrc/gs_bin.h
--- a/3dgs.cpp_amd/csrc/gs_bin.h
+++ b/3dgs.cpp_amd/csrc/gs_bin.h
@@ -180,5 +180,15 @@
     const int lx1 = min((int)box.z, ox + S) - ox - 1, ly1 = min((int)box.w, oy + S) - oy - 1;
     return (uint32_t)lx0 | ((uint32_t)ly0 << 4) | ((uint32_t)lx1 << 8) | ((uint32_t)ly1 << 12);
 }
+constexpr uint32_t kBoxNone = 0xFFFFu;
+__device__ __forceinline__ uint32_t bin_box_pair(const BinGrid& g, uint32_t bin, ushort4 box, ushort4 tight) {
+    const int S = 1 << g.bin_shift;
+    const int ox = (int)(bin & ((1u << g.grid_shift) - 1u)) << g.bin_shift, oy = (int)(bin >> g.grid_shift) << g.bin_shift;
+    const bool hit = max((int)tight.x, ox) < min((int)tight.z, ox + S) && max((int)tight.y, oy) < min((int)tight.w, oy + S);
+    return bin_local_box16(g, bin, box) | ((hit ? bin_local_box16(g, bin, tight) : kBoxNone) << 16);
+}
+__device__ __forceinline__ uint32_t box16_tiles(uint32_t b) {
+    return (((b >> 8) & 15u) - (b & 15u) + 1u) * (((b >> 12) & 15u) - ((b >> 4) & 15u) + 1u);
+}
 
 }
diff --git a/3dgs.cpp_amd/csrc/gs_bin_l1.hip b/3dgs.cpp_amd/csrc/gs_bin_l1.hip
--- a/3dgs.cpp_amd/csrc/gs_bin_l1.hip
+++ b/3dgs.cpp_amd/csrc/gs_bin_l1.hip
@@ -289,7 +289,8 @@
             uint32_t* const rec = a.cand + (size_t)kCandWords * pos;
             rec[0] = k;
             rec[1] = gid;
-            rec[2] = bin_local_box16(a.g, bin, box);
+            const uint32_t b16 = bin_local_box16(a.g, bin, box);
+            rec[2] = b16 | (b16 << 16);
         }
     };
 #pragma unroll
diff --git a/3dgs.cpp_amd/csrc/gs_bin_l2.hip b/3dgs.cpp_amd/csrc/gs_bin_l2.hip
--- a/3dgs.cpp_amd/csrc/gs_bin_l2.hip
+++ b/3dgs.cpp_amd/csrc/gs_bin_l2.hip
@@ -30,6 +30,8 @@
     uint64_t* stamps;
     const uint32_t* l1_words;
     uint32_t l1_cap;
+    uint32_t* bin_count_save;
+    uint32_t reference_boxes;
 };
 
 __device__ __forceinline__ uint32_t bin_candidates(const BuildArgs& a, uint32_t bin) {
@@ -394,7 +396,7 @@
     uint32_t* const t_cnt = smem + 2 * MAXC;
     uint32_t* const t_cur = t_cnt + 64;
     uint32_t (*const s_seg)[64] = reinterpret_cast<uint32_t(*)[64]>(t_cnt + 128);
-    __shared__ uint32_t scratch[NW], scratch_hi[NW];
+    __shared__ uint32_t scratch[NW], scratch_hi[NW], scratch_sum[MODE == 0 ? NW : 1];
     __shared__ uint32_t s_seg0, s_flag;
     constexpr int kSlotBits = SLABS ? 16 : 14;
     constexpr uint32_t kSlotMask = (1u << kSlotBits) - 1u;
@@ -424,6 +426,10 @@
         if (c_total > kMaxInBin) {
             if (tid == 0) atomicOr(&a.counters->overflow, 2u);
             c_total = 0;
+        }
+        if (a.bin_count_save && tid == 0) {
+            a.bin_count_save[bin] = c_total;
+            a.bin_count_save[kBinOffsets + bin] = off;
         }
     };
     if constexpr (MODE == 0 || MODE == 1) bin_extent();
@@ -521,25 +527,32 @@
         }
         __syncthreads();
     };
+    uint32_t ref_mine = 0, ref_inst = 0;
     auto block_minmax = [&](uint32_t lo, uint32_t hi, uint32_t& kmin, uint32_t& span) {
+        uint32_t sum = ref_mine;
 #pragma unroll
         for (int d = 1; d < WAVE; d <<= 1) {
             lo = min(lo, (uint32_t)__shfl_xor((int)lo, d, WAVE));
             hi = max(hi, (uint32_t)__shfl_xor((int)hi, d, WAVE));
+            if constexpr (MODE == 0) sum += (uint32_t)__shfl_xor((int)sum, d, WAVE);
         }
         __syncthreads();
         if (lane == 0) {
             scratch[w] = lo;
             scratch_hi[w] = hi;
-        }
-        __syncthreads();
+            if constexpr (MODE == 0) scratch_sum[w] = sum;
+        }
+        __syncthreads();
+        sum = 0;
 #pragma unroll
         for (int k = 0; k < NW; ++k) {
             lo = min(lo, scratch[k]);
             hi = max(hi, scratch_hi[k]);
+            if constexpr (MODE == 0) sum += scratch_sum[k];
         }
         kmin = (uint32_t)__builtin_amdgcn_readfirstlane((int)lo);
         span = (uint32_t)__builtin_amdgcn_readfirstlane((int)hi) - kmin;
+        if constexpr (MODE == 0) ref_inst = (uint32_t)__builtin_amdgcn_readfirstlane((int)sum);
     };
     auto key_range = [&](uint32_t& kmin, uint32_t& span) {
         uint32_t lo = 0xFFFFFFFFu, hi = 0u;
@@ -660,9 +673,11 @@
         uint32_t d_bin;
         const uint32_t excl = block_excl_scan<THREADS>(v, scratch, &d_bin);
         if (tid == 0) {
-            const uint32_t seg = d_bin ? atomicAdd(&a.counters->instances, d_bin) : 0u;
+            const uint32_t d_ref = MODE == 0 ? ref_inst : d_bin;
+            const uint32_t seg = d_bin ? atomicAdd(&a.counters->listed, d_bin) : 0u;
+            const uint32_t ref_seg = d_ref ? atomicAdd(&a.counters->instances, d_ref) : 0u;
             s_seg0 = seg;
-            if ((uint64_t)seg + d_bin > a.capacity) atomicOr(&a.counters->overflow, 1u);
+            if ((uint64_t)ref_seg + d_ref > a.capacity) atomicOr(&a.counters->overflow, 1u);
         }
         __syncthreads();
         if (tid < 64) {
@@ -888,6 +903,8 @@
         asm volatile("" : "+v"(tid12));
         constexpr int HR = ROUNDS <= 8 ? ROUNDS : ROUNDS / 2;
         const int h_end = multi ? 0 : ROUNDS;
+        const uint32_t box_shift = (MODE == 0 && !a.reference_boxes) ? 16u : 0u;
+        ref_mine = 0;
 #pragma unroll
         for (int h = 0; h < h_end; h += HR) {
             uint32_t k[HR], b[HR];
@@ -906,7 +923,12 @@
                 const uint32_t e = (h + r) * THREADS + tid;
                 if (h + r < rounds && e < c) {
                     s_key[e] = k[r];
-                    s_pay[e] = e | (b[r] << kSlotBits);
+                    if constexpr (MODE == 0) {
+                        s_pay[e] = e | (((b[r] >> box_shift) & 0xFFFFu) << kSlotBits);
+                        ref_mine += box16_tiles(b[r]);
+                    } else {
+                        s_pay[e] = e | (b[r] << kSlotBits);
+                    }
                 }
             }
         }
@@ -981,7 +1003,7 @@
                 const uint32_t pw = s_pay[e];
                 nk[r] = __builtin_amdgcn_raw_buffer_load_b32(recs, (pw & kSlotMask) * 12u, 0, 0);
                 ni[r] = s_id[e] + id_base;
-                nb[r] = pw >> kSlotBits;
+                nb[r] = MODE == 0 ? __builtin_amdgcn_raw_buffer_load_b32(recs, (pw & kSlotMask) * 12u + 8u, 0, 0) : pw >> kSlotBits;
             }
         }
         __syncthreads();
@@ -1311,6 +1333,8 @@
     a.stamps = b.stamps;
     a.l1_words = b.l1_fused_words;
     a.l1_cap = b.l1_fused_cap;
+    a.bin_count_save = b.l1_fused_words ? b.bin_count : nullptr;
+    a.reference_boxes = b.reference_boxes ? 1u : 0u;
     const uint32_t bins = b.bins_x * b.bins_y;
     const bool sort = level < kBinSortLevels;
     if (sort && b.bin_shift <= 3) {
diff --git a/3dgs.cpp_amd/csrc/gs_kernels.h b/3dgs.cpp_amd/csrc/gs_kernels.h
--- a/3dgs.cpp_amd/csrc/gs_kernels.h
+++ b/3dgs.cpp_amd/csrc/gs_kernels.h
@@ -64,6 +64,7 @@
     uint32_t blend_resolved;
     uint32_t blend_redo;
     uint32_t q_head, q_bins_done;
+    uint32_t listed;
 };
 enum FrameStamp { ST_PREPROCESS = 0, ST_ORDER = 1, ST_L1_COUNT = 2, ST_L1_SCATTER = 3, ST_L2 = 4, ST_BLEND = 5, ST_END = 6, ST_COUNT = 8 };
 
@@ -138,6 +139,7 @@
     uint32_t cand_capacity;
     const uint32_t* l1_fused_words;
     uint32_t l1_fused_cap;
+    bool reference_boxes;
     void* slabs;
     uint32_t slab_capacity;
     uint32_t slab_epoch;
diff --git a/3dgs.cpp_amd/csrc/gs_preprocess.hip b/3dgs.cpp_amd/csrc/gs_preprocess.hip
--- a/3dgs.cpp_amd/csrc/gs_preprocess.hip
+++ b/3dgs.cpp_amd/csrc/gs_preprocess.hip
@@ -1,4 +1,5 @@
 #include "gs_bin.h"
+#include "gs_tile_cull.h"
 
 namespace gs {
 
@@ -305,23 +306,28 @@
         for (int k = 0; k < NB / BLOCK; ++k) bins.tbl[k * BLOCK + (int)threadIdx.x] = fbase[k];
         __syncthreads();
         const BinGrid g{lf.tiles_x, lf.tiles_y, lf.bins_x, lf.bins_y, lf.bin_shift, lf.grid_shift};
-        auto emit = [&](uint32_t bin, uint32_t k, uint32_t gid, ushort4 box) {
+        auto emit = [&](uint32_t bin, uint32_t k, uint32_t gid, ushort4 box, ushort4 tight) {
             const uint32_t pos = atomicAdd(&bins.tbl[bin], 1u);
             if (pos < lf.cap) {
                 const uint32_t sb = (bin >> lf.grid_shift) * lf.bins_x + (bin & ((1u << lf.grid_shift) - 1u));
                 uint32_t* const rec = lf.cand + (size_t)kCandWords * ((size_t)sb * lf.cap + pos);
                 rec[0] = k;
                 rec[1] = gid;
-                rec[2] = bin_local_box16(g, bin, box);
+                rec[2] = bin_box_pair(g, bin, box, tight);
             }
         };
         const uint32_t x0 = bb & 255u, y0 = (bb >> 8) & 255u, x1 = (bb >> 16) & 255u, y1 = bb >> 24;
         const ushort4 tb = make_ushort4((unsigned short)bx0, (unsigned short)by0, (unsigned short)bx1, (unsigned short)by1);
+        ushort4 tt = make_ushort4(0, 0, 0, 0);
+        if (vis) {
+            const TileBox t = tile_cull_box(c00, c01, c11, uvx, uvy, acut, TileBox{bx0, by0, bx1, by1});
+            tt = make_ushort4((unsigned short)t.x0, (unsigned short)t.y0, (unsigned short)t.x1, (unsigned short)t.y1);
+        }
         const uint32_t key = __float_as_uint(depth);
         const bool big = (x1 - x0) * (y1 - y0) > kL1BigBox;
         if (!big)
             for (uint32_t y = y0; y < y1; ++y)
-                for (uint32_t x = x0; x < x1; ++x) emit((y << lf.grid_shift) | x, key, oid, tb);
+                for (uint32_t x = x0; x < x1; ++x) emit((y << lf.grid_shift) | x, key, oid, tb, tt);
         for (uint64_t bm = __ballot(big); bm != 0; bm &= bm - 1) {
             const int src = __ffsll((unsigned long long)bm) - 1;
             const uint32_t b1 = (uint32_t)__builtin_amdgcn_readlane((int)bb, src);
@@ -331,7 +337,11 @@
             const uint32_t bhi = (uint32_t)__builtin_amdgcn_readlane((int)((uint32_t)bx1 | ((uint32_t)by1 << 16)), src);
             const ushort4 bbox = make_ushort4((unsigned short)(blo & 0xFFFFu), (unsigned short)(blo >> 16), (unsigned short)(bhi & 0xFFFFu),
                                               (unsigned short)(bhi >> 16));
-            for (uint32_t c = lane; c < cells; c += WAVE) emit(((gy0 + c / bw) << lf.grid_shift) | (gx0 + c % bw), bkey, bgid, bbox);
+            const uint32_t tlo = (uint32_t)__builtin_amdgcn_readlane((int)((uint32_t)tt.x | ((uint32_t)tt.y << 16)), src);
+            const uint32_t thi = (uint32_t)__builtin_amdgcn_readlane((int)((uint32_t)tt.z | ((uint32_t)tt.w << 16)), src);
+            const ushort4 tbox = make_ushort4((unsigned short)(tlo & 0xFFFFu), (unsigned short)(tlo >> 16), (unsigned short)(thi & 0xFFFFu),
+                                              (unsigned short)(thi >> 16));
+            for (uint32_t c = lane; c < cells; c += WAVE) emit(((gy0 + c / bw) << lf.grid_shift) | (gx0 + c % bw), bkey, bgid, bbox, tbox);
         }
     }
 
@@ -389,6 +399,7 @@
         pu.counters->blend_redo = 0;
         pu.counters->q_head = 0;
         pu.counters->q_bins_done = 0;
+        pu.counters->listed = 0;
     }
     preprocess_one<AA, R1>(sv, u, av, i, i < sv.n, s_stage[threadIdx.x / WAVE], lf, s_bins);
 }
diff --git a/3dgs.cpp_amd/csrc/gs_renderer.cpp b/3dgs.cpp_amd/csrc/gs_renderer.cpp
--- a/3dgs.cpp_amd/csrc/gs_renderer.cpp
+++ b/3dgs.cpp_amd/csrc/gs_renderer.cpp
@@ -39,12 +39,12 @@
     hipGraphExec_t graph_execs[2] = {nullptr, nullptr};
     struct GraphKey {
         int level = -1, bin_shift = -1, hw_exp = 0, contract = 1;
-        bool antialiased = false, lockstep = false, l1_fused = false;
+        bool antialiased = false, lockstep = false, l1_fused = false, tile_cull = false;
         uint32_t width = 0, height = 0, capacity = 0, cand_capacity = 0;
         const void *tile_order = nullptr, *ranges = nullptr, *sh16 = nullptr;
         bool operator==(const GraphKey& o) const {
             return level == o.level && bin_shift == o.bin_shift && hw_exp == o.hw_exp && contract == o.contract &&
-                   antialiased == o.antialiased && lockstep == o.lockstep && l1_fused == o.l1_fused &&
+                   antialiased == o.antialiased && lockstep == o.lockstep && l1_fused == o.l1_fused && tile_cull == o.tile_cull &&
                    width == o.width && height == o.height && capacity == o.capacity && cand_capacity == o.cand_capacity &&
                    tile_order == o.tile_order && ranges == o.ranges && sh16 == o.sh16;
         }
@@ -129,6 +129,7 @@
     bool lockstep = false;
     bool l1_fused = false;
     uint32_t l1_cap = 0;
+    bool culled = false;
     uint32_t tune_round = 0;
     int tune_shape = 0;
 };
@@ -148,6 +149,58 @@
     uint32_t default_cand_capacity = 0;
     L1FusedPolicy l1_policy;
     bool last_l1_fused = false;
+    bool tile_cull = !(std::getenv("GS_TILE_CULL") && std::atoi(std::getenv("GS_TILE_CULL")) == 0);
+    bool frame_is_culled(bool l1_fused, int level) const { return tile_cull && l1_fused && level < gs::kBinSlabLevel; }
+    bool last_culled = false;
+    int last_level = 0;
+    BinGeometry last_geo{};
+    uint64_t last_listed = 0;
+    DevBuf<uint32_t> tap_ranges, tap_sorted;
+    DevBuf<gs::Counters> tap_counters;
+    uint64_t tap_frame = ~0ull;
+    const FrameBuffers* tap_set = nullptr;
+    void reference_lists(const uint32_t** ranges, const uint32_t** lists) {
+        FrameBuffers& fb = *last_set;
+        if (!last_culled) {
+            *ranges = fb.ranges.p;
+            *lists = sorted_gid;
+            return;
+        }
+        if (tap_frame != frames_enqueued || tap_set != last_set) {
+            tap_frame = ~0ull;
+            tap_ranges.ensure(2 * num_tiles);
+            tap_sorted.ensure(static_cast<size_t>(capacity) + 4);
+            tap_counters.ensure(1);
+            HIP_CHECK(hipMemsetAsync(tap_counters.p, 0, sizeof(gs::Counters), fb.stream));
+            gs::BinLaunch b{};
+            b.n_bound = static_cast<uint32_t>(scene->n);
+            b.bin_count = fb.bin_count.p;
+            b.cand = fb.cand.p;
+            b.ranges = tap_ranges.p;
+            b.sorted_gid = tap_sorted.p;
+            b.counters = tap_counters.p;
+            b.capacity = capacity;
+            b.cand_capacity = cand_capacity;
+            b.reference_boxes = true;
+            b.tiles_x = tiles_across(last_width);
+            b.tiles_y = tiles_across(last_height);
+            b.bins_x = last_geo.bins_x;
+            b.bins_y = last_geo.bins_y;
+            b.bin_shift = last_geo.bin_shift;
+            b.grid_shift = last_geo.grid_shift;
+            gs::launch_bin_level2(b, last_level, fb.stream);
+            HIP_CHECK(hipGetLastError());
+            gs::Counters c{};
+            HIP_CHECK(hipMemcpyAsync(&c, tap_counters.p, sizeof c, hipMemcpyDeviceToHost, fb.stream));
+            HIP_CHECK(hipStreamSynchronize(fb.stream));
+            if (c.overflow != 0 || c.instances != last.num_instances)
+                throw Error(GS_ERR_DEVICE, "the reference lists of a culled frame do not add up to the frame's instance count");
+            tap_frame = frames_enqueued;
+            tap_set = last_set;
+        }
+        *ranges = tap_ranges.p;
+        *lists = tap_sorted.p;
+    }
     FrameBuffers* last_set = nullptr;
     uint32_t last_width = 0, last_height = 0;
 
@@ -304,6 +357,7 @@
         last_width = last_height = 0;
         num_tiles = 0;
         sorted_gid = depth_order = nullptr;
+        last_culled = false;
     }
     bool has_last_frame() const { return have_frame && last_set != nullptr; }
 
@@ -432,6 +486,7 @@
                 b.cand_capacity = cand_capacity;
                 b.l1_fused_words = lf.words;
                 b.l1_fused_cap = l1_cap;
+                b.reference_boxes = !tile_cull;
                 b.slabs = fb.slabs.p;
                 b.slab_capacity = fb.slabs.p ? gs::kSlabCapacity : 0u;
                 b.slab_epoch = 0;
@@ -464,7 +519,7 @@
             *sl.h_params = gs::FrameParams{u, d_rgba, d_bgra, sl.h_counters, sl.h_stamps};
             HIP_CHECK(hipMemcpyAsync(fb.params.p, sl.h_params, sizeof(gs::FrameParams), hipMemcpyHostToDevice, stream));
             const FrameBuffers::GraphKey key{lv, geo.bin_shift, blend_exp_mode(), contract ? 1 : 0,
-                                             antialiased, lockstep, l1_fused,
+                                             antialiased, lockstep, l1_fused, tile_cull,
                                              u.width, u.height, capacity, cand_capacity,
                                              tile_order.p, fb.ranges.p, sv.sh16};
             const int gi = lockstep ? 1 : 0;
@@ -498,6 +553,9 @@
         last_height = u.height;
         num_tiles = nt;
         last_l1_fused = l1_fused;
+        last_culled = frame_is_culled(l1_fused, lv);
+        last_level = lv;
+        last_geo = geo;
         depth_order = bin_local ? nullptr : fb.dvals[1].p;
         sorted_gid = fb.sorted.p;
 
@@ -506,6 +564,7 @@
         sl.lockstep = lockstep;
         sl.l1_fused = l1_fused;
         sl.l1_cap = l1_cap;
+        sl.culled = frame_is_culled(l1_fused, lv);
         sl.tune_round = tuner.round;
         sl.tune_shape = tune_shape;
         sl.u = u;
@@ -531,6 +590,7 @@
         policy.frame_retired(sl.level, sl.h_counters->max_bin, sl.bin_shift);
         l1_policy.frame_retired(sl.u.width, sl.u.height, sl.bin_shift, sl.h_counters->max_bin, sl.h_counters->bin_entries, sl.h_counters->visible);
         last = frame_stats(sl);
+        last_listed = sl.culled ? sl.h_counters->listed : sl.h_counters->instances;
         have_frame = true;
         const float v[7] = {last.ms_preprocess, last.ms_prefix_sum, last.ms_preprocess_sort, last.ms_sort,
                             last.ms_tile_boundary, last.ms_render, last.ms_total};
@@ -910,6 +970,33 @@
     return rc != 0 ? rc : on;
 }
 
+int gs_set_tile_cull(gs_renderer* r, int enabled) {
+    return guarded([&] {
+        if (!r) throw Error(GS_ERR_INVALID, "null argument");
+        r->drain();
+        r->tile_cull = enabled != 0;
+    });
+}
+
+int gs_get_tile_cull(gs_renderer* r, int* last_frame_culled) {
+    int on = 0;
+    const int rc = guarded([&] {
+        if (!r) throw Error(GS_ERR_INVALID, "null argument");
+        on = r->tile_cull ? 1 : 0;
+        if (last_frame_culled) *last_frame_culled = r->last_set != nullptr && r->last_culled ? 1 : 0;
+    });
+    return rc != 0 ? rc : on;
+}
+
+int gs_get_listed_instances(gs_renderer* r, uint64_t* out) {
+    return guarded([&] {
+        if (!r || !out) throw Error(GS_ERR_INVALID, "null argument");
+        r->drain();
+        if (!r->has_last_frame()) throw Error(GS_ERR_INVALID, "no frame rendered yet");
+        *out = r->last_listed;
+    });
+}
+
 int gs_set_graph_mode(gs_renderer* r, int enabled) {
     return guarded([&] {
         if (!r) throw Error(GS_ERR_INVALID, "renderer is null");
@@ -928,7 +1015,7 @@
         if (stage == GS_STAGE_DEPTH_ORDER && !r->depth_order)
             throw Error(GS_ERR_INVALID, "the depth-order tap exists only on the global depth-order path (gs_set_sort_path(r, 1))");
         const uint64_t n = r->scene->n, v = r->last.num_visible;
-        const uint64_t d = std::min<uint64_t>(r->last.num_instances, r->capacity);
+        const uint64_t d = std::min<uint64_t>(r->last.num_instances, r->capacity), d_ref = d;
         const void* src = nullptr;
         uint64_t size = 0;
         if (r->last_set->planes_stale && (stage == GS_STAGE_TILES || stage == GS_STAGE_DEPTH || stage == GS_STAGE_AABB)) {
@@ -968,10 +1055,18 @@
             case GS_STAGE_SORTED_TILE:
             case GS_STAGE_SORTED_GID:
             case GS_STAGE_RANGES:
+            case GS_STAGE_LISTS_CULLED:
+            case GS_STAGE_RANGES_CULLED:
                 {
+                    const bool own = stage == GS_STAGE_LISTS_CULLED || stage == GS_STAGE_RANGES_CULLED;
+                    const uint32_t *ranges_src = r->last_set->ranges.p, *lists_src = r->sorted_gid;
+                    if (!own) r->reference_lists(&ranges_src, &lists_src);
+                    const uint64_t d = own ? std::min<uint64_t>(r->last_listed, r->capacity) : d_ref;
+                    if (stage == GS_STAGE_RANGES_CULLED) stage = GS_STAGE_RANGES;
+                    if (stage == GS_STAGE_LISTS_CULLED) stage = GS_STAGE_SORTED_GID;
                     const uint64_t nt = r->num_tiles;
                     std::vector<uint32_t> rg(2 * nt);
-                    if (nt) HIP_CHECK(hipMemcpy(rg.data(), r->last_set->ranges.p, rg.size() * 4, hipMemcpyDeviceToHost));
+                    if (nt) HIP_CHECK(hipMemcpy(rg.data(), ranges_src, rg.size() * 4, hipMemcpyDeviceToHost));
                     if (stage == GS_STAGE_RANGES) {
                         if (bytes < nt * 8) throw Error(GS_ERR_INVALID, "destination too small for stage buffer");
                         uint32_t* out = static_cast<uint32_t*>(dst);
@@ -988,7 +1083,7 @@
                     std::vector<uint32_t> lists;
                     if (stage == GS_STAGE_SORTED_GID) {
                         lists.resize(r->capacity);
-                        HIP_CHECK(hipMemcpy(lists.data(), r->sorted_gid, lists.size() * 4, hipMemcpyDeviceToHost));
+                        HIP_CHECK(hipMemcpy(lists.data(), lists_src, lists.size() * 4, hipMemcpyDeviceToHost));
                     }
                     uint32_t* out = static_cast<uint32_t*>(dst);
                     uint64_t pos = 0;
@@ -997,8 +1092,15 @@
                             out[pos++] = stage == GS_STAGE_SORTED_GID ? lists[i] : static_cast<uint32_t>(t);
                     return;
                 }
-            case GS_STAGE_LISTS_RAW: src = r->sorted_gid; size = d * 4; break;
-            case GS_STAGE_RANGES_RAW: src = r->last_set->ranges.p; size = r->num_tiles * 8; break;
+            case GS_STAGE_LISTS_RAW:
+            case GS_STAGE_RANGES_RAW:
+                {
+                    const uint32_t *ranges_src = nullptr, *lists_src = nullptr;
+                    r->reference_lists(&ranges_src, &lists_src);
+                    if (stage == GS_STAGE_LISTS_RAW) src = lists_src, size = d * 4;
+                    else src = ranges_src, size = r->num_tiles * 8;
+                    break;
+                }
             default: throw Error(GS_ERR_INVALID, "unknown stage");
         }
         if (bytes < size) throw Error(GS_ERR_INVALID, "destination too small for stage buffer");
diff --git a/3dgs.cpp_amd/csrc/gs_tile_cull.h b/3dgs.cpp_amd/csrc/gs_tile_cull.h
--- /dev/null
+++ b/3dgs.cpp_amd/csrc/gs_tile_cull.h
@@ -0,0 +1,48 @@
+#pragma once
+#include <cmath>
+#include <cstdint>
+
+#if defined(__HIPCC__) || defined(__CUDACC__)
+#define GS_CULL_HD __host__ __device__ inline
+#else
+#define GS_CULL_HD inline
+#endif
+
+namespace gs {
+
+struct TileBox {
+    int x0, y0, x1, y1;
+};
+
+constexpr int kCullTile = 16;
+constexpr float kCullTermSlack = 9.6e-7f, kCullDetSlack = 1.8e-7f, kCullRelSlack = 4e-6f, kCullAbsSlack = 2.4e-7f;
+
+GS_CULL_HD bool tile_cull_axis(float u, float h, int t0, int t1, int& o0, int& o1) {
+    const float first = (float)(t0 * kCullTile), last = (float)(t1 * kCullTile - 1);
+    const float lo = ceilf(fmaxf(u - h, first)), hi = floorf(fminf(u + h, last));
+    if (lo > hi) return false;
+    o0 = (int)floorf(lo * (1.0f / kCullTile));
+    o1 = (int)floorf(hi * (1.0f / kCullTile)) + 1;
+    return true;
+}
+
+GS_CULL_HD TileBox tile_cull_box(float a, float b, float c, float u, float v, float cut, TileBox ref) {
+    const TileBox none{0, 0, 0, 0};
+    if (cut > 0.0f) return none;
+    if (!(cut > -INFINITY)) return ref;
+    const float ac = a * c, bb = b * b;
+    const float det_lo = (ac - bb) - kCullDetSlack * (ac + bb);
+    if (!(det_lo > 0.0f) || !(a > 0.0f) || !(c > 0.0f) || !(det_lo < INFINITY)) return ref;
+    const float Dx = fmaxf(fabsf(u - (float)(ref.x0 * kCullTile)), fabsf(u - (float)(ref.x1 * kCullTile - 1)));
+    const float Dy = fmaxf(fabsf(v - (float)(ref.y0 * kCullTile)), fabsf(v - (float)(ref.y1 * kCullTile - 1)));
+    const float mag = 0.5f * a * Dx * Dx + 0.5f * c * Dy * Dy + fabsf(b) * Dx * Dy;
+    const float lim = 2.0f * (kCullTermSlack * mag - cut);
+    const float sx = sqrtf(lim * c / det_lo), sy = sqrtf(lim * a / det_lo);
+    const float hx = sx * (1.0f + kCullRelSlack) + (fabsf(u) + sx + 1.0f) * kCullAbsSlack;
+    const float hy = sy * (1.0f + kCullRelSlack) + (fabsf(v) + sy + 1.0f) * kCullAbsSlack;
+    TileBox t;
+    if (!tile_cull_axis(u, hx, ref.x0, ref.x1, t.x0, t.x1) || !tile_cull_axis(v, hy, ref.y0, ref.y1, t.y0, t.y1)) return none;
+    return t;
+}
+
+}
diff --git a/include/gs3d_hip.h b/include/gs3d_hip.h
--- a/include/gs3d_hip.h
+++ b/include/gs3d_hip.h
@@ -74,7 +74,9 @@
     GS_STAGE_SORTED_GID = 12,
     GS_STAGE_RANGES = 13,
     GS_STAGE_LISTS_RAW = 14,
-    GS_STAGE_RANGES_RAW = 15
+    GS_STAGE_RANGES_RAW = 15,
+    GS_STAGE_LISTS_CULLED = 16,
+    GS_STAGE_RANGES_CULLED = 17
 };
 
 const char* gs_last_error(void);
@@ -162,6 +164,9 @@
 int gs_get_blend_lockstep(gs_renderer* r, int* settled);
 int gs_set_level1_fused(gs_renderer* r, int mode);
 int gs_get_level1_fused(gs_renderer* r);
+int gs_set_tile_cull(gs_renderer* r, int enabled);
+int gs_get_tile_cull(gs_renderer* r, int* last_frame_culled);
+int gs_get_listed_instances(gs_renderer* r, uint64_t* out);
 int gs_get_timing_totals(gs_renderer* r, gs_frame_stats* sum, uint64_t* frames, int reset);
 int gs_get_frame_intervals(gs_renderer* r, float* out_ms, uint64_t capacity, uint64_t* n_out, int reset);
 int gs_get_stats(gs_renderer* r, gs_frame_stats* out);
```

New measurement: 5558 (median of 6 runs). +5.4%, better.
